# Aazmp/vp8oclenc

Measured on AMD Instinct MI355X. Metric: macroblocks/sec inter-frame (ME+DCT+loopfilter), 1080p, higher is better.
Workload: dtype u8/int32

## Files before the change

### vp8oclenc_amd/build.py

```python
from __future__ import annotations

import os
import shutil
import subprocess

PKG = os.path.dirname(os.path.abspath(__file__))
CSRC = os.path.join(PKG, "csrc")
LIB = os.path.join(PKG, "libvp8hip.so")
SOURCES = ["api_context.hip", "api_inter.hip", "api_entropy.hip", "api_batch.hip", "api_shard.hip", "api_profile.hip", "kernels_me.hip", "kernels_scale.hip", "kernels_denoise.hip", "api_denoise.hip", "kernels_s2.hip", "kernels_mb.hip", "kernels_lf3.hip", "kernels_lf4.hip", "kernels_lf_simple.hip", "kernels_quality.hip", "api_quality.hip", "kernels_entropy_stage.hip", "kernels_rc.hip", "kernels_intra.hip", "vp8_host.cpp", "vp8_driver.cpp", "vp8_bitstream.cpp"]
HEADERS = ["vp8hip_ctx.h", "vp8hip_dev.h", "kernels_rc_dev.h", "lf_shared.h", "lf_banded.h", "vp8_rfc6386_tables.inc", "vp8_mbhdr.h", "kernels_ent.hip", "kernels_hdr.hip"]
HEADERS = HEADERS + [os.path.join("..", "..", "include", h) for h in ("vp8hip.h", "vp8hip_multi.h", "vp8hip_taps.h", "vp8hip_host.h", "vp8hip_driver.h", "vp8hip_bitstream.h")]


def _hipcc() -> str:
    for cand in (shutil.which("hipcc"), "/opt/rocm/bin/hipcc"):
        if cand and os.path.exists(cand):
            return cand
    raise RuntimeError("hipcc not found: the MI355X path cannot be built (there is no CPU fallback)")


def stale() -> bool:
    if not os.path.exists(LIB):
        return True
    t = os.path.getmtime(LIB)
    deps = [os.path.join(CSRC, s) for s in SOURCES] + [os.path.normpath(os.path.join(CSRC, h)) for h in HEADERS]
    return any(os.path.exists(d) and os.path.getmtime(d) > t for d in deps)


def build(force: bool = False, verbose: bool = False) -> str:
    if not force and not stale():
        return LIB
    objs = []
    procs = []
    odir = os.path.join(PKG, "build")
    os.makedirs(odir, exist_ok=True)
    flags = ["--offload-arch=gfx950", "-O3", "-fPIC", "-std=c++17", "-ffp-contract=off", "-Wall", "-Wno-unused-function", "-Wno-bitwise-instead-of-logical", "-Wno-unused-value", "-Wno-missing-braces",
             "-I", os.path.join(PKG, "..", "include")] + os.environ.get("VP8HIP_EXTRA_FLAGS", "").split()
    for src in SOURCES:
        path = os.path.join(CSRC, src)
        if not os.path.exists(path):
            continue
        obj = os.path.join(odir, os.path.splitext(src)[0] + ".o")
        objs.append(obj)
        cmd = [_hipcc()] + flags + (["-x", "hip"] if src.endswith(".hip") else []) + ["-c", path, "-o", obj]
        if verbose:
            print(" ".join(cmd))
        procs.append((src, subprocess.Popen(cmd, stdout=subprocess.PIPE, stderr=subprocess.STDOUT, text=True)))
    for src, p in procs:
        out, _ = p.communicate()
        if p.returncode != 0:
            raise RuntimeError(f"hipcc failed on {src}:\n{out}")
        if verbose and out.strip():
            print(out)
    cmd = [_hipcc(), "--offload-arch=gfx950", "-shared", "-fPIC", "-o", LIB] + objs + ["-ldl", "-lpthread"]
    r = subprocess.run(cmd, stdout=subprocess.PIPE, stderr=subprocess.STDOUT, text=True)
    if r.returncode != 0:
        raise RuntimeError(f"link failed:\n{r.stdout}")
    return LIB


if __name__ == "__main__":
    print(build(force=True, verbose=True))
```

### vp8oclenc_amd/csrc/api_batch.hip

```cpp
#include "vp8hip_ctx.h"

using namespace vp8;

namespace vp8 {

bool batch_ent_stream(vp8hip_batch *b) {
    static const int mode = [] { const char *v = getenv("VP8HIP_BATCH_ENT_STREAM"); return v && v[0] ? atoi(v) : 0; }();
    if (!b->ev_ent && (hipEventCreateWithFlags(&b->ev_ent_fork, hipEventDisableTiming) != hipSuccess ||
                       hipEventCreateWithFlags(&b->ev_ent, FRAME_EVENT_FLAGS) != hipSuccess))
        return false;
    if (!mode) return false;
    if (b->ent) return true;
    int least = 0, greatest = 0;
    if (mode >= 2 && hipDeviceGetStreamPriorityRange(&least, &greatest) == hipSuccess) {
        if (hipStreamCreateWithPriority(&b->ent, hipStreamNonBlocking, mode == 3 ? greatest : least) != hipSuccess) b->ent = nullptr;
    } else if (hipStreamCreateWithFlags(&b->ent, hipStreamNonBlocking) != hipSuccess) {
        b->ent = nullptr;
    }
    return b->ent != nullptr;
}

}

extern "C" {


int vp8hip_batch_create(vp8hip_batch **out, vp8hip_ctx *const *ctxs, int n) {
    if (!out || !ctxs || n < 1 || n > MAX_BATCH) return VP8HIP_ERR_ARG;
    *out = nullptr;
    for (int i = 0; i < n; ++i) {
        if (!ctxs[i] || ctxs[i]->W != ctxs[0]->W || ctxs[i]->H != ctxs[0]->H || ctxs[i]->device != ctxs[0]->device ||
            ctxs[i]->ssim_target != ctxs[0]->ssim_target || ctxs[i]->lf_overlap || ctxs[i]->conformant != ctxs[0]->conformant ||
            !same_intake(ctxs[i], ctxs[0]))
            return VP8HIP_ERR_ARG;
        if (!ctxs[i]->own_stream) return VP8HIP_ERR_STATE;
        for (int j = 0; j < i; ++j)
            if (ctxs[j] == ctxs[i]) return VP8HIP_ERR_ARG;
    }
    vp8hip_batch *b = new (std::nothrow) vp8hip_batch();
    if (!b) return VP8HIP_ERR_ARG;
    USE_DEVICE(ctxs[0]);
    b->n = n;
    for (int i = 0; i < n; ++i) {
        hipStreamSynchronize(ctxs[i]->stream);
        if (ctxs[i]->own_stream) hipStreamDestroy(ctxs[i]->own_stream);
        ctxs[i]->own_stream = nullptr;
    }
    if (hipStreamCreateWithFlags(&b->stream, hipStreamNonBlocking) != hipSuccess) {
        for (int i = 0; i < n; ++i) {
            hipStreamCreateWithFlags(&ctxs[i]->own_stream, hipStreamNonBlocking);
            ctxs[i]->stream = ctxs[i]->own_stream;
        }
        delete b;
        return VP8HIP_ERR_HIP;
    }
    for (int i = 0; i < n; ++i) {
        ctxs[i]->stream = b->stream;
        ctxs[i]->batch = b;
        b->c[i] = ctxs[i];
        if (ctxs[i]->counted) --g_live_contexts;
        ctxs[i]->counted = false;
    }
    ++g_live_contexts;
    const int prep_mode = vp8hip_batch_prep_mode();
    bool ok = true;
    if (prep_mode) {
        ok = hipEventCreateWithFlags(&b->ev_gate, hipEventDisableTiming) == hipSuccess &&
             hipEventCreateWithFlags(&b->ev_gate2, hipEventDisableTiming) == hipSuccess &&
             hipEventCreateWithFlags(&b->ev_prep, hipEventDisableTiming) == hipSuccess;
        int least = 0, greatest = 0;
        ok = ok && hipDeviceGetStreamPriorityRange(&least, &greatest) == hipSuccess;
        static const bool normal_priority = getenv("VP8HIP_BATCH_PREP_PRIO") != nullptr;
        if (normal_priority) least = 0;
        if (ok && prep_mode == 2) {
            static hipStream_t shared[64] = {};
            hipStream_t &sh = shared[ctxs[0]->device & 63];
            if (!sh) ok = hipStreamCreateWithPriority(&sh, hipStreamNonBlocking, least) == hipSuccess;
            b->prep = sh;
            b->prep_shared = true;
        } else if (ok) {
            ok = hipStreamCreateWithPriority(&b->prep, hipStreamNonBlocking, least) == hipSuccess;
        }
    }
    if (!ok) {
        vp8hip_batch_destroy(b);
        return VP8HIP_ERR_HIP;
    }
    *out = b;
    return VP8HIP_OK;
}

void vp8hip_batch_destroy(vp8hip_batch *b) {
    if (!b) return;
    hipSetDevice(b->c[0]->device);
    if (b->prep) hipStreamSynchronize(b->prep);
    hipStreamSynchronize(b->stream);
    hipStreamDestroy(b->stream);
    if (b->prep && !b->prep_shared) hipStreamDestroy(b->prep);
    if (b->ev_gate) hipEventDestroy(b->ev_gate);
    if (b->ev_gate2) hipEventDestroy(b->ev_gate2);
    if (b->ev_prep) hipEventDestroy(b->ev_prep);
    if (b->ent) {
        hipStreamSynchronize(b->ent);
        hipStreamDestroy(b->ent);
    }
    if (b->copy) {
        hipStreamSynchronize(b->copy);
        hipStreamDestroy(b->copy);
        hipEventDestroy(b->ev_copied);
        hipEventDestroy(b->ev_packed[0]);
        hipEventDestroy(b->ev_packed[1]);
        for (int i = 0; i < b->n; ++i) { hipFree(b->stage[i][0]); hipFree(b->stage[i][1]); }
    }
    if (b->ev_ent_fork) hipEventDestroy(b->ev_ent_fork);
    if (b->ev_ent) hipEventDestroy(b->ev_ent);
    for (int i = 0; i < b->n; ++i) b->c[i]->frame_event = nullptr;
    --g_live_contexts;
    for (int i = 0; i < b->n; ++i) {
        b->c[i]->batch = nullptr;
        if (!b->c[i]->own_stream) hipStreamCreateWithFlags(&b->c[i]->own_stream, hipStreamNonBlocking);
        b->c[i]->stream = b->c[i]->own_stream;
        if (!b->c[i]->counted) ++g_live_contexts;
        b->c[i]->counted = true;
    }
    delete b;
}

static int stage_copy(vp8hip_batch *b, uint8_t *d, const void *y, const void *u, const void *v, size_t ny, size_t nc) {
    vp8hip_ctx *c0 = b->c[0];
    const uint8_t *py = static_cast<const uint8_t *>(y);
    if (u == py + ny && v == py + ny + nc) {
        HIPCHK(c0, hipMemcpyAsync(d, y, ny + 2 * nc, hipMemcpyHostToDevice, b->copy));
        return VP8HIP_OK;
    }
    HIPCHK(c0, hipMemcpyAsync(d, y, ny, hipMemcpyHostToDevice, b->copy));
    HIPCHK(c0, hipMemcpyAsync(d + ny, u, nc, hipMemcpyHostToDevice, b->copy));
    HIPCHK(c0, hipMemcpyAsync(d + ny + nc, v, nc, hipMemcpyHostToDevice, b->copy));
    return VP8HIP_OK;
}

static int batch_stage_ready(vp8hip_batch *b) {
    vp8hip_ctx *c0 = b->c[0];
    int sw, sh;
    incoming_size(c0, &sw, &sh);
    const size_t bytes = (size_t)sw * sh + 2 * (size_t)(sw / 2) * (sh / 2);
    if (!b->copy) {
        HIPCHK(c0, hipStreamCreateWithFlags(&b->copy, hipStreamNonBlocking));
        HIPCHK(c0, hipEventCreateWithFlags(&b->ev_copied, hipEventDisableTiming));
        HIPCHK(c0, hipEventCreateWithFlags(&b->ev_packed[0], hipEventDisableTiming));
        HIPCHK(c0, hipEventCreateWithFlags(&b->ev_packed[1], hipEventDisableTiming));
    }
    if (b->stage_bytes == bytes) return VP8HIP_OK;
    HIPCHK(c0, hipStreamSynchronize(b->copy));
    HIPCHK(c0, hipStreamSynchronize(b->stream));
    if (b->prep) HIPCHK(c0, hipStreamSynchronize(b->prep));
    for (int i = 0; i < b->n; ++i)
        for (int k = 0; k < 2; ++k) {
            (void)hipFree(b->stage[i][k]);
            b->stage[i][k] = nullptr;
            HIPCHK(c0, hipMalloc(&b->stage[i][k], bytes));
        }
    b->stage_bytes = bytes;
    b->packed_valid[0] = b->packed_valid[1] = false;
    b->pre_valid = false;
    return VP8HIP_OK;
}

static int batch_set_current(vp8hip_batch *b, const int *active, const void *const *y, const void *const *u, const void *const *v, bool host) {
    if (!b || !y || !u || !v) return VP8HIP_ERR_ARG;
    vp8hip_ctx *c0 = b->c[0];
    USE_DEVICE_ONLY(c0);
    const void *sy[MAX_BATCH], *su[MAX_BATCH], *sv[MAX_BATCH];
    int slot = -1;
    for (int i = 0; i < b->n; ++i) {
        if (active && !active[i]) continue;
        if (!y[i] || !u[i] || !v[i]) return VP8HIP_ERR_ARG;
        if (!same_intake(b->c[i], c0)) return VP8HIP_ERR_ARG;
    }
    if (host) {
        const int rc = batch_stage_ready(b);
        if (rc) return rc;
        int sw, sh;
        incoming_size(c0, &sw, &sh);
        const size_t ny = (size_t)sw * sh, nc = (size_t)(sw / 2) * (sh / 2);
        slot = b->stage_idx ^= 1;
        bool waited = false;
        for (int i = 0; i < b->n; ++i) {
            if (active && !active[i]) continue;
            uint8_t *d = b->stage[i][slot];
            if (!(b->pre_valid && b->pre[i][0] == y[i] && b->pre[i][1] == u[i] && b->pre[i][2] == v[i])) {
                if (!waited && b->packed_valid[slot]) HIPCHK(c0, hipStreamWaitEvent(b->copy, b->ev_packed[slot], 0));
                waited = true;
                {
                    const int cr = stage_copy(b, d, y[i], u[i], v[i], ny, nc);
                    if (cr) {
                        b->stage_idx ^= 1;
                        b->pre_valid = false;
                        return cr;
                    }
                }
            }
            sy[i] = d; su[i] = d + ny; sv[i] = d + ny + nc;
        }
        b->pre_valid = false;
        HIPCHK(c0, hipEventRecord(b->ev_copied, b->copy));
        y = sy; u = su; v = sv;
    }
    const Frame *f[MAX_BATCH];
    const void *py[MAX_BATCH], *pu[MAX_BATCH], *pv[MAX_BATCH];
    const ScalePlan *plans[MAX_BATCH];
    int n = 0;
    for (int i = 0; i < b->n; ++i) {
        if (active && !active[i]) continue;
        flush_scan(b->c[i]);
        next_current(b->c[i]);
        f[n] = &b->c[i]->cur;
        plans[n] = &b->c[i]->scale;
        py[n] = y[i]; pu[n] = u[i]; pv[n] = v[i];
        ++n;
    }
    if (!n) return VP8HIP_OK;
    hipStream_t ps = b->stream;
    if (b->prep) {
        HIPCHK(c0, hipStreamWaitEvent(b->prep, b->ev_gate, 0));
        HIPCHK(c0, hipEventRecord(b->ev_gate2, b->stream));
        hipEvent_t t_ = b->ev_gate;
        b->ev_gate = b->ev_gate2;
        b->ev_gate2 = t_;
        b->prep_pending = true;
        ps = b->prep;
    }
    if (host) HIPCHK(c0, hipStreamWaitEvent(ps, b->ev_copied, 0));
    {
        Timed t(c0, VP8HIP_K_PACK);
        if (c0->scale.in_w) launch_scale_batch(ps, f, py, pu, pv, plans, n);
        else launch_pack_batch(ps, f, py, pu, pv, n, c0->src_w, c0->src_h);
    }
    {
        DenoiseItem dn[MAX_BATCH];
        int nd = 0;
        for (int i = 0; i < b->n; ++i) {
            if (active && !active[i]) continue;
            if (denoise_item(b->c[i], ps, dn[nd])) ++nd;
        }
        launch_denoise_batch(ps, dn, nd, c0->dn_level);
    }
    HIPCHK(c0, hipGetLastError());
    if (host) {
        HIPCHK(c0, hipEventRecord(b->ev_packed[slot], ps));
        b->packed_valid[slot] = true;
    }
    return VP8HIP_OK;
}

int vp8hip_batch_set_current_device(vp8hip_batch *b, const int *active, const void *const *y, const void *const *u, const void *const *v) {
    return batch_set_current(b, active, y, u, v, false);
}

int vp8hip_batch_prefetch_current(vp8hip_batch *b, const uint8_t *const *y, const uint8_t *const *u, const uint8_t *const *v) {
    if (!b || !y || !u || !v) return VP8HIP_ERR_ARG;
    vp8hip_ctx *c0 = b->c[0];
    USE_DEVICE_ONLY(c0);
    const int rc = batch_stage_ready(b);
    if (rc) return rc;
    int sw, sh;
    incoming_size(c0, &sw, &sh);
    const size_t ny = (size_t)sw * sh, nc = (size_t)(sw / 2) * (sh / 2);
    const int slot = b->stage_idx ^ 1;
    if (b->packed_valid[slot]) HIPCHK(c0, hipStreamWaitEvent(b->copy, b->ev_packed[slot], 0));
    for (int i = 0; i < b->n; ++i) {
        b->pre[i][0] = b->pre[i][1] = b->pre[i][2] = nullptr;
        if (!y[i] || !u[i] || !v[i]) continue;
        uint8_t *d = b->stage[i][slot];
        { const int cr = stage_copy(b, d, y[i], u[i], v[i], ny, nc); if (cr) return cr; }
        b->pre[i][0] = y[i]; b->pre[i][1] = u[i]; b->pre[i][2] = v[i];
    }
    HIPCHK(c0, hipEventRecord(b->ev_copied, b->copy));
    b->pre_valid = true;
    return VP8HIP_OK;
}

int vp8hip_batch_upload_current(vp8hip_batch *b, const int *active, const uint8_t *const *y, const uint8_t *const *u, const uint8_t *const *v) {
    if (!b) return VP8HIP_ERR_ARG;
    if (b->copy) {
        (void)hipSetDevice(b->c[0]->device);
        HIPCHK(b->c[0], hipEventSynchronize(b->ev_copied));
    }
    return batch_set_current(b, active, reinterpret_cast<const void *const *>(y), reinterpret_cast<const void *const *>(u),
                             reinterpret_cast<const void *const *>(v), true);
}

int vp8hip_batch_auto_segments(vp8hip_batch *b, const int *active, const int *is_key_frame, const int32_t (*refqi)[4], int qi_min) {
    if (!b || !is_key_frame || !refqi) return VP8HIP_ERR_ARG;
    vp8hip_ctx *c0 = b->c[0];
    USE_DEVICE_ONLY(c0);
    const Frame *cur[MAX_BATCH];
    uint32_t *partial[MAX_BATCH], *stats[MAX_BATCH];
    SegData *sd[MAX_BATCH];
    int32_t *strength[MAX_BATCH];
    int key[MAX_BATCH];
    int32_t qi[MAX_BATCH][4];
    int n = 0;
    for (int i = 0; i < b->n; ++i) {
        if (active && !active[i]) continue;
        vp8hip_ctx *c = b->c[i];
        if (c->cur_count == 0) return VP8HIP_ERR_STATE;
        next_params(c);
        cur[n] = &c->cur;
        partial[n] = c->d_stats + 8;
        stats[n] = c->d_stats;
        sd[n] = c->d_sd;
        strength[n] = reinterpret_cast<int32_t *>(c->d_stats + 4);
        key[n] = is_key_frame[i] ? 1 : 0;
        for (int k = 0; k < 4; ++k) qi[n][k] = refqi[i][k];
        ++n;
    }
    static const bool own_launch = [] { const char *v = getenv("VP8HIP_BATCH_SCAN_LAUNCH"); return v && v[0] == '1'; }();
    if (n && !b->prep && !own_launch) {
        int k = 0;
        for (int i = 0; i < b->n; ++i) {
            if (active && !active[i]) continue;
            vp8hip_ctx *c = b->c[i];
            c->scan_req = ScanRequest{partial[k], stats[k], sd[k], strength[k], key[k], {qi[k][0], qi[k][1], qi[k][2], qi[k][3]}, qi_min};
            c->scan_deferred = true;
            ++k;
        }
        return VP8HIP_OK;
    }
    if (n && b->prep) b->prep_pending = true;
    if (n) launch_auto_segments_batch(b->prep ? b->prep : b->stream, cur, partial, stats, sd, strength, key, qi, qi_min, n);
    HIPCHK(c0, hipGetLastError());
    return VP8HIP_OK;
}

int vp8hip_batch_inter_transform(vp8hip_batch *b, const int *active, const int *prev_is_golden, const int *prev_is_altref,
                                 const int *use_golden, const int *use_altref) {
    if (!b || !prev_is_golden || !prev_is_altref || !use_golden || !use_altref) return VP8HIP_ERR_ARG;
    vp8hip_ctx *c0 = b->c[0];
    USE_DEVICE_ONLY(c0);
    vp8hip_ctx *m[MAX_BATCH];
    RefSet refs[MAX_BATCH];
    const Frame *cur[MAX_BATCH], *recon[MAX_BATCH], *pyr[2 * MAX_BATCH], *pyr_cur[MAX_BATCH];
    const ScanRequest *scans[MAX_BATCH] = {};
    int npyr_cur = 0;
    const NetSet *nets[MAX_BATCH];
    const MBOut *outs[MAX_BATCH];
    const SegData *sds[MAX_BATCH];
    int n = 0, npyr = 0;
    uint32_t pyr_border = 0;
    for (int i = 0; i < b->n; ++i) {
        if (active && !active[i]) continue;
        if (b->c[i]->conformant != c0->conformant) return VP8HIP_ERR_ARG;
        const int rc = inter_check(b->c[i], prev_is_golden[i], prev_is_altref[i], use_golden[i], use_altref[i]);
        if (rc) return rc;
    }
    for (int i = 0; i < b->n; ++i) {
        if (active && !active[i]) continue;
        vp8hip_ctx *c = b->c[i];
        const int rc = inter_begin(c, prev_is_golden[i], prev_is_altref[i], use_golden[i], use_altref[i]);
        if (rc) {
            for (int k = 0; k < n; ++k)
                if (scans[k]) m[k]->scan_deferred = true;
            return rc;
        }
        FrameSurf &last = c->frames[c->slot[0]];
        if (!c->cur_pyramid_valid) {
            if (b->prep) pyr_cur[npyr_cur++] = &c->cur;
            else pyr[npyr++] = &c->cur;
        }
        bool border_alone = false;
        if (!last.pyramid_valid) {
            if (!last.border_valid) pyr_border |= 1u << npyr;
            pyr[npyr++] = &last.f;
        } else if (!last.border_valid) {
            border_alone = true;
        }
        if (border_alone) {
            batch_join_prep(b);
            launch_border(b->stream, last.f);
        }
        last.pyramid_valid = true;
        last.border_valid = true;
        c->cur_pyramid_valid = true;
        refs[n] = ref_set(c, 1, use_golden[i], use_altref[i]);
        cur[n] = &c->cur;
        recon[n] = &c->frames[c->recon].f;
        nets[n] = &c->nets;
        outs[n] = &c->out;
        sds[n] = c->d_sd;
        if (c->scan_deferred) {
            scans[n] = &c->scan_req;
            c->scan_deferred = false;
        }
        m[n++] = c;
    }
    if (!n) return VP8HIP_OK;
    hipStream_t s = b->stream;
    if (npyr_cur) {
        b->prep_pending = true;
        launch_pyramid_batch(b->prep, pyr_cur, npyr_cur, 0);
    }
    batch_join_prep(b);
    if (npyr) {
        Timed t(c0, VP8HIP_K_DOWNSAMPLE);
        launch_pyramid_batch(s, pyr, npyr, pyr_border);
    }
    const int net_width = c0->mbw * 2;
    static const int coarse_mode = [] { const char *v = getenv("VP8HIP_BATCH_S1_COARSE"); return v && v[0] ? atoi(v) : 0; }();
    int first_level = 4, src = 0;
    if (coarse_mode > 0 && c0->mbw >= 2 && c0->mbh >= 2) {
        Timed t(c0, VP8HIP_K_SEARCH1_L2);
        if (launch_search1_coarse_batch(s, cur, refs, nets, net_width, n, coarse_mode == 2, coarse_mode == 3)) {
            first_level = coarse_mode == 2 ? -1 : (coarse_mode == 3 ? 1 : 0);
            src = first_level == 1 ? 1 : 0;
        }
    }
    for (int l = first_level; l >= 0; --l) {
        Timed t(c0, VP8HIP_K_SEARCH1_L4 + (4 - l));
        launch_search1_batch(s, cur, refs, nets, l, src, net_width, n);
        src ^= 1;
    }
    bool carried;
    {
        Timed t(c0, VP8HIP_K_SEARCH2);
        carried = launch_search2_batch(s, cur, refs, nets, n, s2_clock(c0), scans);
    }
    for (int i = 0; i < n && !carried; ++i)
        if (scans[i]) launch_auto_segments(s, m[i]->cur, scans[i]->partial, scans[i]->stats, scans[i]->sd, scans[i]->strength_out, scans[i]->is_key,
                                           scans[i]->refqi, scans[i]->qi_min);
    {
        Timed t(c0, VP8HIP_K_MB);
        launch_mb_batch(s, cur, refs, nets, recon, outs, sds, c0->ssim_target, c0->mbw, c0->mbh, n, c0->conformant != 0);
    }
    for (int i = 0; i < n; ++i) m[i]->recon_ready = true, m[i]->recon_key = false;
    HIPCHK(c0, hipGetLastError());
    return VP8HIP_OK;
}

int vp8hip_batch_loop_filter(vp8hip_batch *b, const int *active) {
    if (!b) return VP8HIP_ERR_ARG;
    vp8hip_ctx *c0 = b->c[0];
    USE_DEVICE(c0);
    vp8hip_ctx *m[MAX_BATCH];
    const Frame *recon[MAX_BATCH];
    const MBOut *outs[MAX_BATCH];
    SegData *sds[MAX_BATCH];
    int32_t *prog[MAX_BATCH];
    void *hand[MAX_BATCH];
    unsigned launch_no[MAX_BATCH];
    LfCheck chk[MAX_BATCH];
    int n = 0, type = -1;
    for (int i = 0; i < b->n; ++i) {
        if (active && !active[i]) continue;
        if (!b->c[i]->recon_ready || b->c[i]->recon < 0) return VP8HIP_ERR_STATE;
        if (type >= 0 && b->c[i]->lf_type != type) return VP8HIP_ERR_STATE;
        type = b->c[i]->lf_type;
    }
    for (int i = 0; i < b->n; ++i) {
        if (active && !active[i]) continue;
        vp8hip_ctx *c = b->c[i];
        recon[n] = &c->frames[c->recon].f;
        outs[n] = &c->out;
        sds[n] = c->d_sd;
        prog[n] = c->d_progress;
        hand[n] = c->d_lf_handoff;
        launch_no[n] = type == 1 ? c->lf_simple_launches++ : c->lf_launches++;
        lf_check(c, chk[n]);
        c->verdict_stream = b->stream;
        m[n++] = c;
    }
    if (!n) return VP8HIP_OK;
    if (b->ent) HIPCHK(c0, hipEventRecord(b->ev_ent_fork, b->stream));
    {
        Timed t(c0, VP8HIP_K_LOOP_FILTER);
        static const bool form4 = [] { const char *v = getenv("VP8HIP_LF_BATCH_FORM"); return v && atoi(v) == 4; }();
        if (type == 1) launch_loop_filter_simple_batch(b->stream, recon, outs, sds, prog, c0->mbw, c0->mbh, launch_no, n, chk);
        else if (form4) launch_loop_filter4_batch(b->stream, recon, outs, sds, prog, hand, c0->mbw, c0->mbh, launch_no, n, chk);
        else launch_loop_filter3_batch(b->stream, recon, outs, sds, prog, c0->mbw, c0->mbh, launch_no, n, chk);
    }
    b->ent_fork_fresh = b->ent != nullptr;
    for (int i = 0; i < n; ++i) {
        vp8hip_ctx *c = m[i];
        c->frames[c->recon].pyramid_valid = false;
        c->frames[c->recon].border_valid = false;
        c->slot[0] = c->recon;
        c->lf_key = c->recon_key;
        c->recon = -1;
        c->recon_ready = false;
    }
    HIPCHK(c0, hipGetLastError());
    return batch_quality(b, active);
}

int vp8hip_batch_intra_transform(vp8hip_batch *b, const int *active) {
    if (!b) return VP8HIP_ERR_ARG;
    vp8hip_ctx *c0 = b->c[0];
    USE_DEVICE(c0);
    for (int i = 0; i < b->n; ++i) {
        if (active && !active[i]) continue;
        if (b->c[i]->cur_count == 0) return VP8HIP_ERR_STATE;
    }
    CheckItem it[MAX_BATCH];
    vp8hip_ctx *m[MAX_BATCH];
    int n = 0;
    for (int i = 0; i < b->n; ++i) {
        if (active && !active[i]) continue;
        vp8hip_ctx *c = b->c[i];
        const int rc = claim_recon(c);
        if (rc) return rc;
        c->ent_counted_partitions = 0;
        drop_overflowed_frame(c);
        ++c->out_gen;
        CheckItem &k = it[n];
        k.cur = &c->cur;
        k.recon = &c->frames[c->recon].f;
        k.o = &c->out;
        k.sd = c->d_sd;
        k.modes = c->intra_modes;
        k.is_inter = c->intra_is_inter;
        k.prog = c->intra_prog;
        k.err = c->d_progress + LF_ERR_WORD;
        k.gen = ++c->intra_gen;
        m[n++] = c;
    }
    if (!n) return VP8HIP_OK;
    {
        Timed t(c0, VP8HIP_K_INTRA);
        launch_intra_key_batch(b->stream, it, n, c0->mbw, c0->mbh);
    }
    {
        Timed t(c0, VP8HIP_K_FILTER_MASK);
        for (int i = 0; i < n; ++i) launch_filter_mask(b->stream, m[i]->out, m[i]->d_sd, m[i]->mbs);
    }
    for (int i = 0; i < n; ++i) m[i]->recon_ready = true, m[i]->recon_key = true;
    HIPCHK(c0, hipGetLastError());
    return VP8HIP_OK;
}

int vp8hip_batch_check_ssim_async(vp8hip_batch *b, const int *active, const int32_t (*refqi)[4], int qi_min) {
    if (!b || !refqi) return VP8HIP_ERR_ARG;
    vp8hip_ctx *c0 = b->c[0];
    USE_DEVICE(c0);
    for (int i = 0; i < b->n; ++i) {
        if (active && !active[i]) continue;
        const vp8hip_ctx *c = b->c[i];
        if (!c->recon_ready || c->recon < 0 || c->cur_count == 0 || c->verdict_pending || c->chk_armed) return VP8HIP_ERR_STATE;
    }
    CheckItem it[MAX_BATCH];
    int n = 0;
    for (int i = 0; i < b->n; ++i) {
        if (active && !active[i]) continue;
        check_item(b->c[i], it[n++], refqi[i], qi_min);
    }
    if (!n) return VP8HIP_OK;
    if (fallback_possible(c0->ssim_target)) {
        Timed t(c0, VP8HIP_K_INTRA);
        launch_check_fallback(b->stream, it, n, c0->ssim_target, c0->mbw, c0->mbh, c0->conformant);
    }
    HIPCHK(c0, hipGetLastError());
    return VP8HIP_OK;
}

int vp8hip_batch_encode_frame_begin(vp8hip_batch *b, const int *active, int num_partitions, const vp8hip_header_params *params) {
    if (!b || !params) return VP8HIP_ERR_ARG;
    const int P = num_partitions;
    if (P != 1 && P != 2 && P != 4 && P != 8) return VP8HIP_ERR_ARG;
    vp8hip_ctx *c0 = b->c[0];
    bool early = b->ent_fork_fresh;
    USE_DEVICE(c0);
    FrameEntropy e[MAX_BATCH];
    FrameOut fo[MAX_BATCH];
    vp8hip_ctx *m[MAX_BATCH];
    int n = 0;
    for (int i = 0; i < b->n; ++i) {
        if (active && !active[i]) continue;
        if (b->c[i]->frame_pending) return VP8HIP_ERR_STATE;
    }
    for (int i = 0; i < b->n; ++i) {
        if (active && !active[i]) continue;
        vp8hip_ctx *c = b->c[i];
        const int rc = frame_prepare(c, P, &params[i], e[n], fo[n]);
        if (rc) return rc;
        c->frame_params = params[i];
        c->frame_partitions = P;
        m[n++] = c;
    }
    if (!n) return VP8HIP_OK;
    const bool side = !c0->prof_mask && batch_ent_stream(b);
    hipStream_t s = side ? b->ent : b->stream;
    if (side) {
        for (int i = 0; i < n; ++i) early = early && !m[i]->verdict_pending;
        if (!early) HIPCHK(c0, hipEventRecord(b->ev_ent_fork, b->stream));
        HIPCHK(c0, hipStreamWaitEvent(b->ent, b->ev_ent_fork, 0));
    }
    {
        Timed t(c0, VP8HIP_K_ENT_COUNT);
        launch_fe_count_batch(s, e, n);
    }
    {
        Timed t(c0, VP8HIP_K_HDR_ENCODE);
        launch_fe_emit_batch(s, e, n);
    }
    {
        Timed t(c0, VP8HIP_K_ENT_ENCODE);
        launch_frame_code_batch(s, e, fo, n);
    }
    HIPCHK(c0, hipGetLastError());
    for (int i = 0; i < n; ++i) {
        vp8hip_ctx *c = m[i];
        c->ent_counted_partitions = P;
        if (!frame_zero_copy()) {
            const size_t first = c->h_frame_cap < FRAME_FIRST_COPY ? c->h_frame_cap : FRAME_FIRST_COPY;
            HIPCHK(c0, hipMemcpyAsync(c->h_frame, c->d_frame, first, hipMemcpyDeviceToHost, s));
        }
        c->frame_pending = true;
        c->frame_gen = c->out_gen;
        c->frame_event = b->ev_ent;
    }
    if (b->ev_ent) HIPCHK(c0, hipEventRecord(b->ev_ent, s));
    if (side) HIPCHK(c0, hipStreamWaitEvent(b->stream, b->ev_ent, 0));
    return VP8HIP_OK;
}

}
```

### vp8oclenc_amd/csrc/api_profile.hip

```cpp
#include "vp8hip_ctx.h"

using namespace vp8;

namespace vp8 {

int prof_collect(vp8hip_ctx *c) {
    if (c->ev_used == 0) return VP8HIP_OK;
    HIPCHK(c, hipStreamSynchronize(c->stream));
    for (int i = 0; i < c->ev_used; i += 2) {
        float ms = 0;
        HIPCHK(c, hipEventElapsedTime(&ms, c->ev[i], c->ev[i + 1]));
        c->prof_ms[c->ev_kernel[i / 2]] += ms;
        c->prof_n[c->ev_kernel[i / 2]] += 1;
    }
    c->ev_used = 0;
    return VP8HIP_OK;
}

}

extern "C" {

int vp8hip_profile_enable(vp8hip_ctx *c, uint32_t mask) {
    USE_DEVICE(c);
    JOIN_LF(c);
    if (!c) return VP8HIP_ERR_ARG;
    int rc = prof_collect(c);
    c->prof_mask = mask;
    return rc;
}

int vp8hip_profile_read(vp8hip_ctx *c, double *total_ms, int64_t *launches) {
    USE_DEVICE(c);
    if (!c) return VP8HIP_ERR_ARG;
    int rc = prof_collect(c);
    if (rc) return rc;
    for (int k = 0; k < VP8HIP_K_COUNT; ++k) {
        if (total_ms) total_ms[k] = c->prof_ms[k];
        if (launches) launches[k] = c->prof_n[k];
        c->prof_ms[k] = 0;
        c->prof_n[k] = 0;
    }
    return VP8HIP_OK;
}

int vp8hip_profile_read_clock(vp8hip_ctx *c, double *loop_filter_ms, int64_t *loop_filter_launches, double *shader_clock_ghz) {
    USE_DEVICE(c);
    if (!c || !loop_filter_ms || !loop_filter_launches) return VP8HIP_ERR_ARG;
    JOIN_LF(c);
    unsigned long long clk[6] = {0, 0, 0, 0, 0, 0};
    int32_t *base = c->d_progress + LF_ERR_WORD + 4;
    HIPCHK(c, hipMemcpyAsync(clk, base, sizeof(clk), hipMemcpyDeviceToHost, c->stream));
    HIPCHK(c, hipMemsetAsync(base + 2, 0, 40, c->stream));
    HIPCHK(c, hipStreamSynchronize(c->stream));
    c->lf_context_switches = (int64_t)clk[5];
    if (getenv("VP8HIP_DEBUG_CLOCK")) fprintf(stderr, "lf clock: launches %llu anomalies %llu hw_id changed %llu\n", clk[2], clk[4], clk[5]);
    *loop_filter_ms = (double)clk[1] * 1e-5;
    *loop_filter_launches = (int64_t)clk[2];
    if (shader_clock_ghz) *shader_clock_ghz = clk[2] > clk[4] ? (double)clk[3] / (double)(clk[2] - clk[4]) * 1e-4 : 0.0;
    return VP8HIP_OK;
}

int vp8hip_profile_search2_clock(vp8hip_ctx *c, int on) {
    if (!c) return VP8HIP_ERR_ARG;
    c->s2_clock_on = on != 0;
    return VP8HIP_OK;
}

int vp8hip_profile_read_search2_clock(vp8hip_ctx *c, double *ms, int64_t *launches) {
    USE_DEVICE(c);
    if (!c || !ms || !launches) return VP8HIP_ERR_ARG;
    JOIN_LF(c);
    unsigned long long w[5] = {0, 0, 0, 0, 0};
    HIPCHK(c, hipMemcpyAsync(w, s2_clock_words(c), sizeof(w), hipMemcpyDeviceToHost, c->stream));
    HIPCHK(c, hipMemsetAsync(s2_clock_words(c) + 3, 0, 16, c->stream));
    HIPCHK(c, hipStreamSynchronize(c->stream));
    *ms = (double)w[3] * 1e-5;
    *launches = (int64_t)w[4];
    return VP8HIP_OK;
}

int64_t vp8hip_profile_context_switches(const vp8hip_ctx *c) { return c ? c->lf_context_switches : 0; }

int vp8hip_debug_download(vp8hip_ctx *c, int what, int ref, int level, void *dst, size_t bytes) {
    USE_DEVICE(c);
    JOIN_LF(c);
    if (!c || !dst) return VP8HIP_ERR_ARG;
    hipStream_t s = c->stream;
    switch (what) {
        case VP8HIP_DBG_NET1:
        case VP8HIP_DBG_NET2: {
            if (ref < 0 || ref > 2 || bytes != (size_t)c->b8 * 4) return VP8HIP_ERR_ARG;
            HIPCHK(c, hipMemcpyAsync(dst, c->nets.net[ref][what == VP8HIP_DBG_NET1 ? 0 : 1], bytes, hipMemcpyDeviceToHost, s));
            break;
        }
        case VP8HIP_DBG_BDIFF:
            if (ref < 0 || ref > 2 || bytes != (size_t)c->b8 * 4) return VP8HIP_ERR_ARG;
            HIPCHK(c, hipMemcpyAsync(dst, c->nets.bdiff[ref], bytes, hipMemcpyDeviceToHost, s));
            break;
        case VP8HIP_DBG_PYRAMID: {
            if (ref < 0 || ref > 3 || level < 0 || level > 4) return VP8HIP_ERR_ARG;
            if (ref < 3 && c->slot[ref] < 0) return VP8HIP_ERR_STATE;
            const Frame &f = ref == 3 ? c->cur : c->frames[c->slot[ref]].f;
            const Plane &p = f.Y[level];
            if (bytes != (size_t)p.w * p.h) return VP8HIP_ERR_ARG;
            int rc = copy_out(c, dst, p);
            if (rc) return rc;
            break;
        }
        case VP8HIP_DBG_MB_MASK:
        case VP8HIP_DBG_MB_NZ:
            if (bytes != (size_t)c->mbs * 4) return VP8HIP_ERR_ARG;
            HIPCHK(c, hipMemcpyAsync(dst, what == VP8HIP_DBG_MB_MASK ? c->out.mask : c->out.nz, bytes, hipMemcpyDeviceToHost, s));
            break;
        case VP8HIP_DBG_THIRD_CONTEXT:
            if (bytes != (size_t)c->mbs * 25) return VP8HIP_ERR_ARG;
            HIPCHK(c, hipMemcpyAsync(dst, c->ent_third, bytes, hipMemcpyDeviceToHost, s));
            break;
        case VP8HIP_DBG_CURRENT_CHROMA: {
            if (ref < 0 || ref > 1 || c->cur_count == 0) return VP8HIP_ERR_ARG;
            const Plane &p = ref ? c->cur.V : c->cur.U;
            if (bytes != (size_t)p.w * p.h) return VP8HIP_ERR_ARG;
            int rc = copy_out(c, dst, p);
            if (rc) return rc;
            break;
        }
        case 100:
            if (bytes != 512) return VP8HIP_ERR_ARG;
            HIPCHK(c, hipMemcpyAsync(dst, (const char *)c->d_progress + 4096, 512, hipMemcpyDeviceToHost, s));
            break;
        default:
            return VP8HIP_ERR_ARG;
    }
    HIPCHK(c, hipStreamSynchronize(s));
    return VP8HIP_OK;
}

int vp8hip_debug_weight(vp8hip_ctx *c, const int32_t *d, int n, int32_t *out) {
    USE_DEVICE(c);
    JOIN_LF(c);
    if (!c || !d || !out || n <= 0) return VP8HIP_ERR_ARG;
    int32_t *dd = nullptr, *dout = nullptr;
    HIPCHK(c, hipMalloc(&dd, (size_t)n * 64));
    HIPCHK(c, hipMalloc(&dout, (size_t)n * 4));
    HIPCHK(c, hipMemcpyAsync(dd, d, (size_t)n * 64, hipMemcpyHostToDevice, c->stream));
    launch_weight_tap(c->stream, dd, n, dout);
    HIPCHK(c, hipMemcpyAsync(out, dout, (size_t)n * 4, hipMemcpyDeviceToHost, c->stream));
    HIPCHK(c, hipStreamSynchronize(c->stream));
    hipFree(dd);
    hipFree(dout);
    return VP8HIP_OK;
}

int vp8hip_debug_weight_mfma(vp8hip_ctx *c, const int32_t *d, int n, int32_t *out) {
    USE_DEVICE(c);
    JOIN_LF(c);
    if (!c || !d || !out || n <= 0) return VP8HIP_ERR_ARG;
    int32_t *dd = nullptr, *dout = nullptr;
    HIPCHK(c, hipMalloc(&dd, (size_t)n * 64));
    HIPCHK(c, hipMalloc(&dout, (size_t)n * 4));
    HIPCHK(c, hipMemcpyAsync(dd, d, (size_t)n * 64, hipMemcpyHostToDevice, c->stream));
    launch_weight_tap_mfma(c->stream, dd, n, dout);
    HIPCHK(c, hipMemcpyAsync(out, dout, (size_t)n * 4, hipMemcpyDeviceToHost, c->stream));
    HIPCHK(c, hipStreamSynchronize(c->stream));
    hipFree(dd);
    hipFree(dout);
    return VP8HIP_OK;
}

int vp8hip_debug_lf_stall(vp8hip_ctx *c, int on) {
    USE_DEVICE(c);
    JOIN_LF(c);
    if (!c) return VP8HIP_ERR_ARG;
    c->lf_stall_test = on ? 1 : 0;
    return VP8HIP_OK;
}

int vp8hip_debug_upload_ssim(vp8hip_ctx *c, const float *ssim) {
    USE_DEVICE(c);
    JOIN_LF(c);
    if (!c || !ssim) return VP8HIP_ERR_ARG;
    HIPCHK(c, hipMemcpyAsync(c->out.ssim, ssim, (size_t)c->mbs * 4, hipMemcpyHostToDevice, c->stream));
    HIPCHK(c, hipStreamSynchronize(c->stream));
    return VP8HIP_OK;
}

int vp8hip_debug_upload_header_inputs(vp8hip_ctx *c, const int32_t *seg, const int32_t *nz, const int32_t *ref, const int32_t *parts,
                                      const int16_t *vectors, const int32_t *is_inter, const int32_t *modes, const uint32_t *probs,
                                      const uint32_t *denom, const int32_t *sd) {
    USE_DEVICE(c);
    JOIN_LF(c);
    if (!c) return VP8HIP_ERR_ARG;
    hipStream_t s = c->stream;
    const size_t n = c->mbs;
    if (seg) HIPCHK(c, hipMemcpyAsync(c->out.seg, seg, n * 4, hipMemcpyHostToDevice, s));
    if (nz) HIPCHK(c, hipMemcpyAsync(c->out.nz, nz, n * 4, hipMemcpyHostToDevice, s));
    if (ref) HIPCHK(c, hipMemcpyAsync(c->out.ref, ref, n * 4, hipMemcpyHostToDevice, s));
    if (parts) HIPCHK(c, hipMemcpyAsync(c->out.parts, parts, n * 4, hipMemcpyHostToDevice, s));
    if (vectors) HIPCHK(c, hipMemcpyAsync(c->out.vec, vectors, n * 16, hipMemcpyHostToDevice, s));
    if (is_inter) HIPCHK(c, hipMemcpyAsync(c->intra_is_inter, is_inter, n * 4, hipMemcpyHostToDevice, s));
    if (modes) HIPCHK(c, hipMemcpyAsync(c->intra_modes, modes, n * 64, hipMemcpyHostToDevice, s));
    if (probs) HIPCHK(c, hipMemcpyAsync(c->ent_probs, probs, sizeof(uint32_t) * ENT_NCTX, hipMemcpyHostToDevice, s));
    if (denom) HIPCHK(c, hipMemcpyAsync(c->ent_denom0, denom, sizeof(uint32_t) * ENT_NCTX, hipMemcpyHostToDevice, s));
    if (sd) HIPCHK(c, hipMemcpyAsync(c->d_sd, sd, sizeof(SegData), hipMemcpyHostToDevice, s));
    HIPCHK(c, hipStreamSynchronize(s));
    if (probs || denom) c->ent_counted_partitions = 1;
    return VP8HIP_OK;
}

}
```

### vp8oclenc_amd/csrc/kernels_lf3.hip

```cpp
#include "lf_banded.h"

namespace vp8 {

namespace lf3 {

using namespace lfb;

struct NormalFilter {
    static constexpr bool CHROMA = true;
    static constexpr bool LEVEL0_ENDS_PLANE = true;
    typedef int4 Lim;
    static __device__ __forceinline__ Lim limits(const int32_t *sd) {
        const int il = sd[SD_INTERIOR_LIMIT] & 0xff;
        return make_int4(il, il - (sd[SD_MBEDGE_LIMIT] & 0xff) * 2 - 1, il - (sd[SD_SUB_BEDGE_LIMIT] & 0xff) * 2 - 1, sd[SD_HEV_THRESHOLD] & 0xff);
    }
    struct Step { Limits L; int int_lim, il4, il8; };
    static __device__ __forceinline__ Step step(const Lim &lim, bool inner, bool luma) {
        Step s;
        s.int_lim = lim.x;
        s.L.mb_delta = lim.y;
        s.L.b_delta = lim.z;
        s.L.hev_thr = lim.w;
        s.il4 = inner ? s.int_lim : -1;
        s.il8 = inner && luma ? s.int_lim : -1;
        return s;
    }
    static __device__ __forceinline__ void line(int (&t)[20], const Step &s, bool mb_edge) { filter_line(t, s.L, mb_edge ? s.int_lim : -1, s.il4, s.il8); }
};

__global__ __launch_bounds__(NWAVES * 64) void k_loop_filter3_b(BatchOf<Args> b) { loop_filter_body<NormalFilter>(b.item[blockIdx.z]); }

}

static bool lf_skip() {
    static const bool skip = experiment_skip("lf");
    return skip;
}

void launch_loop_filter3_batch(hipStream_t s, const Frame *const *recon, const MBOut *const *o, SegData *const *d_sd,
                               int32_t *const *progress, int mbw, int mbh, const unsigned *launch_no, int n, const LfCheck *chk) {
    lfb::launch_batch(lf3::k_loop_filter3_b, s, recon, o, d_sd, progress, 0, mbw, mbh, launch_no, n, chk, lf_skip());
}

}
```

### vp8oclenc_amd/csrc/kernels_lf_simple.hip

```cpp
#include "lf_banded.h"

namespace vp8 {

namespace lfs {

using namespace lfb;

__device__ __forceinline__ void simple_edge(int &p0, int &q0, int p1, int q1, int lim2) {
    const int sum = (int)__builtin_amdgcn_sad_u16((uint32_t)p1, (uint32_t)q1, (uint32_t)(ad(p0, q0) << 2));
    int w = c128(c128(p1 - q1) + __mul24(q0 - p0, 3));
    w = sum <= lim2 ? w : 0;
    w = imin(w, 123);
    q0 = satb(q0 - ((w + 4) >> 3));
    p0 = satb(p0 + ((w + 3) >> 3));
}

__device__ __forceinline__ void simple_line(int (&t)[20], int lim2_mb, int lim2_in) {
#pragma unroll
    for (int k = 4; k < 20; k += 4) simple_edge(t[k - 1], t[k], t[k - 2], t[k + 1], k == 4 ? lim2_mb : lim2_in);
}

struct SimpleFilter {
    static constexpr bool CHROMA = false;
    static constexpr bool LEVEL0_ENDS_PLANE = false;
    typedef int2 Lim;
    static __device__ __forceinline__ Lim limits(const int32_t *sd) {
        const bool on = sd[SD_LOOP_FILTER_LEVEL] != 0;
        return make_int2(on ? (sd[SD_MBEDGE_LIMIT] & 0xff) * 2 + 1 : -1, on ? (sd[SD_SUB_BEDGE_LIMIT] & 0xff) * 2 + 1 : -1);
    }
    struct Step { int lim_mb, lim_in; };
    static __device__ __forceinline__ Step step(const Lim &lim, bool inner, bool) { return Step{lim.x, inner ? lim.y : -1}; }
    static __device__ __forceinline__ void line(int (&t)[20], const Step &s, bool mb_edge) { simple_line(t, mb_edge ? s.lim_mb : -1, s.lim_in); }
};

__global__ __launch_bounds__(NWAVES * 64) void k_loop_filter_simple(Args a) { loop_filter_body<SimpleFilter>(a); }
__global__ __launch_bounds__(NWAVES * 64) void k_loop_filter_simple_b(BatchOf<Args> b) { loop_filter_body<SimpleFilter>(b.item[blockIdx.z]); }

}

bool loop_filter_simple_fits(int mbh) { return (mbh + 1 + lfb::ROWS - 1) / lfb::ROWS + 1 <= LF_SIMPLE_WORDS; }

void launch_loop_filter_simple(hipStream_t s, const Frame &recon, const MBOut &o, SegData *d_sd, int32_t *progress, int mbw, int mbh,
                               unsigned launch_no, const LfCheck *chk) {
    const lfb::Args a = lfb::make_args(s, recon, o, d_sd, progress, LF_SIMPLE_WORD, mbw, mbh, launch_no, chk);
    VP8_LAUNCH(lfs::k_loop_filter_simple, dim3(a.nbands + (a.chk.on ? 1 : 0)), dim3(lfb::NWAVES * 64), 0, s, a);
}

void launch_loop_filter_simple_batch(hipStream_t s, const Frame *const *recon, const MBOut *const *o, SegData *const *d_sd,
                                     int32_t *const *progress, int mbw, int mbh, const unsigned *launch_no, int n, const LfCheck *chk) {
    lfb::launch_batch(lfs::k_loop_filter_simple_b, s, recon, o, d_sd, progress, LF_SIMPLE_WORD, mbw, mbh, launch_no, n, chk);
}

}
```

### vp8oclenc_amd/csrc/kernels_me.hip

```cpp
#include <stdlib.h>
#include <string.h>

#include "vp8hip_dev.h"

namespace vp8 {

struct BorderItem { Plane y, u, v; };
static_assert(EXT == 8, "border_row stores a margin as one eight-byte word");
__device__ __forceinline__ void border_row(const Plane &pl, int row, int lane) {
    if (row >= pl.h + EXT) return;
    uint8_t *dst = pl.p + (ptrdiff_t)row * pl.stride;
    const uint8_t *src = pl.p + (ptrdiff_t)iclamp(row, 0, pl.h - 1) * pl.stride;
    if (row < 0 || row >= pl.h)
        for (int x = lane * 8; x < pl.w; x += 512) *reinterpret_cast<uint2 *>(dst + x) = *reinterpret_cast<const uint2 *>(src + x);
    if (lane < 2) {
        const uint32_t s4 = (uint32_t)src[lane ? pl.w - 1 : 0] * 0x01010101u;
        *reinterpret_cast<uint2 *>(dst + (lane ? pl.w : -EXT)) = make_uint2(s4, s4);
    }
}
__device__ __forceinline__ void border_body(const BorderItem &a) {
    border_row(blockIdx.y == 0 ? a.y : (blockIdx.y == 1 ? a.u : a.v), (int)blockIdx.x - EXT, threadIdx.x);
}

__global__ __launch_bounds__(64) void k_border(BorderItem a) { border_body(a); }

void launch_border(hipStream_t s, const Frame &f) {
    dim3 grid(f.Y[0].h + 2 * EXT, 3);
    VP8_LAUNCH(k_border, grid, dim3(64), 0, s, BorderItem{f.Y[0], f.U, f.V});
}

struct PyrArgs { Frame f[2 * MAX_BATCH]; uint32_t border_mask; };
static int border_jobs(const Frame &f) { return (f.Y[0].h + 2 * EXT) + 2 * (f.U.h + 2 * EXT); }

__global__ __launch_bounds__(256) void k_pyramid(PyrArgs a) {
    __shared__ uint8_t s2[16][16];
    __shared__ uint8_t s3[8][8];
    const Frame &f = a.f[blockIdx.z];
    const int t = threadIdx.x, tx = t & 15, ty = t >> 4;
    const Plane &P0 = f.Y[0];
    const int tiles_y = (P0.h + 63) / 64;
    const int tile = xcd_band((int)blockIdx.y * (int)gridDim.x + (int)blockIdx.x, tiles_y * (int)gridDim.x);
    const int bx = tile % (int)gridDim.x, by = tile / (int)gridDim.x;
    if ((int)blockIdx.y >= tiles_y) {
        if (!((a.border_mask >> blockIdx.z) & 1)) return;
        int job = (((int)blockIdx.y - tiles_y) * (int)gridDim.x + (int)blockIdx.x) * 4 + (t >> 6);
        const int ny = P0.h + 2 * EXT, nc = f.U.h + 2 * EXT;
        if (job < ny) border_row(P0, job - EXT, t & 63);
        else if (job < ny + nc) border_row(f.U, job - ny - EXT, t & 63);
        else if (job < ny + 2 * nc) border_row(f.V, job - ny - nc - EXT, t & 63);
        return;
    }
    const int sx = imin(bx * 64 + 4 * tx, P0.w - 4), sy0 = by * 64 + 4 * ty;
    uint32_t r[4];
#pragma unroll
    for (int k = 0; k < 4; ++k)
        r[k] = *reinterpret_cast<const uint32_t *>(P0.p + (ptrdiff_t)imin(sy0 + k, P0.h - 1) * P0.stride + sx);
    int l1[2][2];
#pragma unroll
    for (int j = 0; j < 2; ++j)
#pragma unroll
        for (int i = 0; i < 2; ++i)
            l1[j][i] = (byte_of(r[2 * j], 2 * i) + byte_of(r[2 * j], 2 * i + 1) + byte_of(r[2 * j + 1], 2 * i) +
                        byte_of(r[2 * j + 1], 2 * i + 1) + 2) >> 2;
    const Plane &P1 = f.Y[1];
    const int x1 = bx * 32 + 2 * tx, y1 = by * 32 + 2 * ty;
    if (x1 < P1.w) {
#pragma unroll
        for (int j = 0; j < 2; ++j)
            if (y1 + j < P1.h)
                *reinterpret_cast<uint16_t *>(P1.p + (ptrdiff_t)(y1 + j) * P1.stride + x1) = (uint16_t)(l1[j][0] | (l1[j][1] << 8));
    }
    const int l2 = (l1[0][0] + l1[0][1] + l1[1][0] + l1[1][1] + 2) >> 2;
    const Plane &P2 = f.Y[2];
    const int x2 = bx * 16 + tx, y2 = by * 16 + ty;
    if (x2 < P2.w && y2 < P2.h) P2.p[(ptrdiff_t)y2 * P2.stride + x2] = (uint8_t)l2;
    s2[ty][tx] = (uint8_t)l2;
    __syncthreads();
    if (t < 64) {
        const int ux = t & 7, uy = t >> 3;
        const int l3 = (s2[2 * uy][2 * ux] + s2[2 * uy][2 * ux + 1] + s2[2 * uy + 1][2 * ux] + s2[2 * uy + 1][2 * ux + 1] + 2) >> 2;
        const Plane &P3 = f.Y[3];
        const int x3 = bx * 8 + ux, y3 = by * 8 + uy;
        if (x3 < P3.w && y3 < P3.h) P3.p[(ptrdiff_t)y3 * P3.stride + x3] = (uint8_t)l3;
        s3[uy][ux] = (uint8_t)l3;
    }
    __syncthreads();
    if (t < 16) {
        const int ux = t & 3, uy = t >> 2;
        const int l4 = (s3[2 * uy][2 * ux] + s3[2 * uy][2 * ux + 1] + s3[2 * uy + 1][2 * ux] + s3[2 * uy + 1][2 * ux + 1] + 2) >> 2;
        const Plane &P4 = f.Y[4];
        const int x4 = bx * 4 + ux, y4 = by * 4 + uy;
        if (x4 < P4.w && y4 < P4.h) P4.p[(ptrdiff_t)y4 * P4.stride + x4] = (uint8_t)l4;
    }
}

static dim3 pyramid_grid(const Frame &f, int nframes, uint32_t border_mask) {
    const int gx = (f.Y[0].w + 63) / 64, gy = (f.Y[0].h + 63) / 64;
    const int extra = border_mask ? ((border_jobs(f) + 3) / 4 + gx - 1) / gx : 0;
    return dim3(gx, gy + extra, nframes);
}
void launch_pyramid(hipStream_t s, const Frame *a, const Frame *b, uint32_t border_mask) {
    PyrArgs p;
    p.f[0] = *a;
    p.f[1] = b ? *b : *a;
    p.border_mask = border_mask;
    VP8_LAUNCH(k_pyramid, pyramid_grid(*a, b ? 2 : 1, border_mask), dim3(256), 0, s, p);
}
void launch_pyramid_batch(hipStream_t s, const Frame *const *f, int nframes, uint32_t border_mask) {
    if (nframes <= 0) return;
    PyrArgs p;
    for (int i = 0; i < nframes; ++i) p.f[i] = *f[i];
    p.border_mask = border_mask;
    VP8_LAUNCH(k_pyramid, pyramid_grid(*f[0], nframes, border_mask), dim3(256), 0, s, p);
}

struct PackItem { Plane py, pu, pv; const uint8_t *sy, *su, *sv; int sw, sh, ssy, ssc; };
__device__ __forceinline__ void pack_body(const PackItem &a, int per) {
    const Plane &py = a.py, &pu = a.pu, &pv = a.pv;
    const uint8_t *sy = a.sy, *su = a.su, *sv = a.sv;
    const int ny = (py.w >> 3) * py.h, nc = (pu.w >> 3) * pu.h;
    for (int k = 0; k < per; ++k) {
        int i = ((int)blockIdx.x * per + k) * 256 + (int)threadIdx.x;
        const Plane *pl = &py;
        const uint8_t *src = sy;
        int sw = a.sw, sh = a.sh, ss = a.ssy;
        if (i >= ny) {
            i -= ny;
            pl = &pu;
            src = su;
            sw >>= 1; sh >>= 1; ss = a.ssc;
            if (i >= nc) { i -= nc; pl = &pv; src = sv; }
            if (i >= nc) return;
        }
        const int upr = pl->w >> 3;
        const int y = i / upr, x = (i % upr) * 8;
        const uint8_t *row = src + (size_t)(y < sh ? y : sh - 1) * ss;
        uint2 v;
        if (x + 8 <= sw && ((ss | (int)(reinterpret_cast<uintptr_t>(src) & 7)) & 7) == 0) {
            v = *reinterpret_cast<const uint2 *>(row + x);
        } else {
            uint32_t w[2] = {0, 0};
#pragma unroll
            for (int j = 0; j < 8; ++j) w[j >> 2] |= (uint32_t)row[x + j < sw ? x + j : sw - 1] << (8 * (j & 3));
            v = make_uint2(w[0], w[1]);
        }
        *reinterpret_cast<uint2 *>(pl->p + (ptrdiff_t)y * pl->stride + x) = v;
    }
}

__global__ __launch_bounds__(256) void k_pack_b(BatchOf<PackItem> b, int per) { pack_body(b.item[blockIdx.z], per); }
static int pack_units_per_thread() {
    static const int per = [] { const char *e = getenv("VP8HIP_PACK_UNITS"); const int v = e ? atoi(e) : 16; return v < 1 ? 1 : (v > 64 ? 64 : v); }();
    return per;
}

static PackItem pack_item(const Frame &f, const void *y, const void *u, const void *v, int sw, int sh, int ssy, int ssc) {
    if (sw <= 0) { sw = f.Y[0].w; sh = f.Y[0].h; }
    if (ssy <= 0) { ssy = sw; ssc = sw >> 1; }
    return PackItem{f.Y[0], f.U, f.V, (const uint8_t *)y, (const uint8_t *)u, (const uint8_t *)v, sw, sh, ssy, ssc};
}
void launch_pack(hipStream_t s, const Frame &f, const void *y, const void *u, const void *v, int sw, int sh, int ssy, int ssc) {
    const int n = (f.Y[0].w >> 3) * f.Y[0].h + 2 * ((f.U.w >> 3) * f.U.h);
    BatchOf<PackItem> b;
    b.n = 1;
    b.item[0] = pack_item(f, y, u, v, sw, sh, ssy, ssc);
    const int per = pack_units_per_thread();
    VP8_LAUNCH(k_pack_b, dim3((n + 256 * per - 1) / (256 * per), 1, 1), dim3(256), 0, s, b, per);
}
void launch_pack_batch(hipStream_t s, const Frame *const *f, const void *const *y, const void *const *u, const void *const *v, int n,
                       int sw, int sh) {
    BatchOf<PackItem> b;
    b.n = n;
    for (int i = 0; i < n; ++i) b.item[i] = pack_item(*f[i], y[i], u[i], v[i], sw, sh, 0, 0);
    const int units = (f[0]->Y[0].w >> 3) * f[0]->Y[0].h + 2 * ((f[0]->U.w >> 3) * f[0]->U.h);
    static const bool skip = experiment_skip("pack");
    if (skip) return;
    const int per = pack_units_per_thread();
    VP8_LAUNCH(k_pack_b, dim3((units + 256 * per - 1) / (256 * per), 1, n), dim3(256), 0, s, b, per);
}

struct Search1Args {
    Plane cur;
    Plane ref[3];
    const int16_t *src[3];
    int16_t *dst[3];
    int refmap[3];
    int nrefs;
    int net_width, w, h, pixel_rate, rate_shift, nblk, bw;
    int pbw, pbh;
    uint32_t bw_inv;
};

template <bool SPLIT>
struct S1Map {
    static constexpr int LANES_PER_BLOCK = SPLIT ? 20 : 5;
    static constexpr int BLOCKS_PER_WAVE = SPLIT ? 3 : 12;
    static constexpr int BLOCKS_PER_WG = 4 * BLOCKS_PER_WAVE;
};

__device__ __forceinline__ void s1_subblock(const uint8_t *cp, int cstride, const uint8_t *rp, int rstride, int acc[5]) {
    uint32_t c[4], q0[4], q1[4];
#pragma unroll
    for (int y = 0; y < 4; ++y) {
        c[y] = *reinterpret_cast<const uint32_t *>(cp + (ptrdiff_t)y * cstride) ^ 0x80808080u;
        const uint2 q = ld_u64(rp + (ptrdiff_t)y * rstride);
        q0[y] = q.x ^ 0x80808080u; q1[y] = q.y ^ 0x80808080u;
    }
    uint32_t cc[4], col[8];
    transpose4x4(c, cc);
    transpose4x4(q0, col);
    transpose4x4(q1, col + 4);
    int pre[16];
#pragma unroll
    for (int k = 0; k < 4; ++k) weight_pre_column(cc[k], pre + 4 * k);
#pragma unroll
    for (int i = 0; i < 5; ++i) acc[i] += weight_cols_pre(pre, col + i);
}

__device__ __forceinline__ int vcopy(uint32_t x) {
    int y;
    asm volatile("v_mov_b32 %0, %1" : "=v"(y) : "v"(x));
    return y;
}
__device__ __forceinline__ void s1_subblock_pre(v4i wa, const int *pre_lds, int pre_off, const uint8_t *rp, int rstride, int acc[5]) {
    uint32_t q0[4], q1[4];
#pragma unroll
    for (int y = 0; y < 4; ++y) {
        const uint2 q = ld_u64(rp + (ptrdiff_t)y * rstride);
        q0[y] = q.x ^ 0x80808080u; q1[y] = q.y ^ 0x80808080u;
    }
    uint32_t col[8];
    transpose4x4(q0, col);
    transpose4x4(q1, col + 4);
#pragma unroll
    for (int i = 0; i < 5; ++i) {
        int off = pre_off;
        asm volatile("" : "+v"(off));
        __builtin_amdgcn_sched_barrier(0);
        const v4i b = (i & 1) ? v4i{vcopy(col[i]), vcopy(col[i + 1]), vcopy(col[i + 2]), vcopy(col[i + 3])}
                              : v4i{(int)col[i], (int)col[i + 1], (int)col[i + 2], (int)col[i + 3]};
        acc[i] += weight_mfma(wa, load_pre16(pre_lds + off), b);
    }
}
constexpr int S1_PRE_INTS = 12 * 4 * 16;
__device__ __forceinline__ void s1_make_pre(const Plane &cur, int cx, int cy, int sb, bool on, int *dst16) {
    const int sx = (sb >> 1) * 4, sy = (sb & 1) * 4;
    const uint8_t *cp = cur.p + (ptrdiff_t)(cy + sy) * cur.stride + cx + sx;
    uint32_t c[4], cc[4];
#pragma unroll
    for (int y = 0; y < 4; ++y) c[y] = *reinterpret_cast<const uint32_t *>(cp + (ptrdiff_t)y * cur.stride) ^ 0x80808080u;
    transpose4x4(c, cc);
    int pre[16];
    weight_pre_block(cc, pre);
    if (on) {
#pragma unroll
        for (int k = 0; k < 4; ++k) *reinterpret_cast<int4 *>(dst16 + 4 * k) = make_int4(pre[4 * k], pre[4 * k + 1], pre[4 * k + 2], pre[4 * k + 3]);
    }
}

template <bool SPLIT, bool PRE_LDS = false>
__device__ __forceinline__ uint32_t search1_block(const Search1Args &a, int r, int cx, int cy, uint32_t pv, bool live, int sub, int lane,
                                                  const int *pre_lds = nullptr ,
                                                  int pre_off = 0 ) {
    const int sb0 = sub / 5, j = sub - 5 * sb0;
    int v0x = (int16_t)(pv & 0xffffu), v0y = (int16_t)(pv >> 16);
    const int rmask = a.pixel_rate - 1;
    v0x = (v0x + ((v0x >> 31) & rmask)) >> a.rate_shift;
    v0y = (v0y + ((v0y >> 31) & rmask)) >> a.rate_shift;
    if (a.pixel_rate > 8) v0x = v0y = 0;

    const int py = (int16_t)(cy + v0y + (j - 2));
    const bool row_valid = live && py >= 0 && py <= a.h - 8;
    const int xb = cx + v0x - 2;
    const bool loadable = row_valid && xb >= -8 && xb <= a.w - 4;
    const int lx = loadable ? xb : cx, ly = loadable ? py : cy;

    const uint8_t *cp = a.cur.p + (ptrdiff_t)cy * a.cur.stride + cx;
    const uint8_t *rp = a.ref[r].p + (ptrdiff_t)ly * a.ref[r].stride + lx;
    int acc[5] = {0, 0, 0, 0, 0};
    if (SPLIT) {
        const int sx = (sb0 >> 1) * 4, sy = (sb0 & 1) * 4;
        s1_subblock(cp + (ptrdiff_t)sy * a.cur.stride + sx, a.cur.stride, rp + (ptrdiff_t)sy * a.ref[r].stride + sx, a.ref[r].stride, acc);
#pragma unroll
        for (int i = 0; i < 5; ++i) {
            acc[i] += __shfl(acc[i], lane + 10, 64);
            acc[i] += __shfl(acc[i], lane + 5, 64);
        }
    } else {
        if (PRE_LDS) {
            const v4i wa = metric_a(lane);
#pragma unroll 1
            for (int sb = 0; sb < 4; ++sb) {
                const int sx = (sb >> 1) * 4, sy = (sb & 1) * 4;
                s1_subblock_pre(wa, pre_lds, pre_off + 16 * sb, rp + (ptrdiff_t)sy * a.ref[r].stride + sx, a.ref[r].stride, acc);
            }
        } else {
#pragma unroll 1
            for (int sb = 0; sb < 4; ++sb) {
                const int sx = (sb >> 1) * 4, sy = (sb & 1) * 4;
                s1_subblock(cp + (ptrdiff_t)sy * a.cur.stride + sx, a.cur.stride, rp + (ptrdiff_t)sy * a.ref[r].stride + sx, a.ref[r].stride, acc);
            }
        }
    }
    const int pen_mask = a.pixel_rate < 4 ? -1 : 0;
    const int pen_y = iabs(iabs(py - cy) - v0y);
    uint32_t best = 0xffffffffu;
#pragma unroll
    for (int i = 0; i < 5; ++i) {
        const int px = (int16_t)(xb + i);
        const bool valid = loadable && px >= 0 && px <= a.w - 8;
        const int diff = (acc[i] + (((iabs(iabs(px - cx) - v0x) + pen_y) << 5) & pen_mask)) & 0xffff;
        const uint32_t key = (valid && diff < 0x7fff) ? ((uint32_t)diff << 8) | (uint32_t)(j * 5 + i) : 0xffffffffu;
        best = key < best ? key : best;
    }
#pragma unroll
    for (int off = 1; off <= 4; off <<= 1) {
        const uint32_t o = (uint32_t)__shfl((int)best, lane + off, 64);
        if (j + off < 5 && o < best) best = o;
    }
    int bx, by;
    if (best != 0xffffffffu) {
        const int k = best & 0xff;
        bx = v0x + (k % 5 - 2);
        by = v0y + (k / 5 - 2);
    } else {
        bx = (int16_t)(v0x - cx);
        by = (int16_t)(v0y - cy);
    }
    const uint32_t ox16 = (uint16_t)(int16_t)((int16_t)bx * (int16_t)a.pixel_rate);
    const uint32_t oy16 = (uint16_t)(int16_t)((int16_t)by * (int16_t)a.pixel_rate);
    return ox16 | (oy16 << 16);
}

template <bool SPLIT, bool PRE_LDS = false, bool REF_LOOP = false>
__device__ __forceinline__ void search1_body(const Search1Args &a) {
    using M = S1Map<SPLIT>;
    if (!REF_LOOP && (int)blockIdx.y >= a.nrefs) return;
    const int lane = threadIdx.x & 63, wave = threadIdx.x >> 6;
    const int grp = lane / M::LANES_PER_BLOCK, sub = lane - M::LANES_PER_BLOCK * grp;
    const int b_raw = (xcd_band(blockIdx.x, gridDim.x) * 4 + wave) * M::BLOCKS_PER_WAVE + grp;
    const bool live = grp < M::BLOCKS_PER_WAVE && b_raw < a.nblk;
    const int b = live ? b_raw : a.nblk - 1;
    const int by = a.bw == 1 ? b : (int)__umulhi((uint32_t)b, a.bw_inv), bx = b - by * a.bw;
    const int cx = bx * 8, cy = by * 8;
    const int parent = (cy >> 4) * a.net_width + (cx >> 4);
    const bool parent_written = (cx >> 4) < a.pbw && (cy >> 4) < a.pbh;
    const int *pre_lds = nullptr;
    int pre_off = 0;
    if (!SPLIT && PRE_LDS) {
        __shared__ __attribute__((aligned(16))) int s_pre[4][S1_PRE_INTS];
        const int slot = lane >> 2, sb = lane & 3;
        const int tb_raw = (xcd_band(blockIdx.x, gridDim.x) * 4 + wave) * M::BLOCKS_PER_WAVE + slot;
        const int tb = tb_raw < a.nblk ? tb_raw : a.nblk - 1;
        const int tby = a.bw == 1 ? tb : (int)__umulhi((uint32_t)tb, a.bw_inv), tbx = tb - tby * a.bw;
        s1_make_pre(a.cur, tbx * 8, tby * 8, sb, slot < M::BLOCKS_PER_WAVE, &s_pre[wave][(slot < M::BLOCKS_PER_WAVE ? slot : 0) * 64 + sb * 16]);
        asm volatile("s_waitcnt lgkmcnt(0)" ::: "memory");
        pre_lds = &s_pre[0][0];
        pre_off = wave * S1_PRE_INTS + (grp < M::BLOCKS_PER_WAVE ? grp : 0) * 64;
    }
    const int nr = REF_LOOP ? a.nrefs : 1;
#pragma unroll 1
    for (int ri = 0; ri < nr; ++ri) {
        const int r = a.refmap[REF_LOOP ? ri : (int)blockIdx.y];
        const uint32_t pv = parent_written ? reinterpret_cast<const uint32_t *>(a.src[r])[parent] : 0u;
        const uint32_t out = search1_block<SPLIT, !SPLIT && PRE_LDS>(a, r, cx, cy, pv, live, sub, lane, pre_lds, pre_off);
        if (sub == 0 && live) {
            const int cell = (cy >> 3) * a.net_width + (cx >> 3);
            reinterpret_cast<uint32_t *>(a.dst[r])[cell] = out;
        }
    }
}

struct CoarseArgs { Search1Args lv[5]; };
constexpr int COARSE_WAVES = 6;
template <bool FINEST, bool TOP_ONLY = false>
__device__ __forceinline__ void coarse_tile(const Search1Args &L0, const Search1Args &L1, const Search1Args &L2, const Search1Args &L3, const Search1Args &L4, int r) {
    using M = S1Map<true>;
    __shared__ uint32_t mv4, mv3, mv2[4], mv1[16];
    const int lane = threadIdx.x & 63, wave = threadIdx.x >> 6;
    const int grp = lane / M::LANES_PER_BLOCK, sub = lane - M::LANES_PER_BLOCK * grp;
    const int slot = grp < M::BLOCKS_PER_WAVE ? wave * M::BLOCKS_PER_WAVE + grp : 99;
    const int tiles_x = (L1.bw + 3) / 4;
    const int tile = xcd_band(blockIdx.x, gridDim.x);
    const int ty = tile / tiles_x, tx = tile - ty * tiles_x;
    {
        const int bx = tx >> 1, by = ty >> 1;
        const bool exists = bx < L4.bw && by * L4.bw + bx < L4.nblk;
        if (wave == 0) {
            const bool live = slot == 0 && exists;
            const uint32_t out = search1_block<true>(L4, r, (live ? bx : 0) * 8, (live ? by : 0) * 8, 0u, live, sub, lane);
            if (slot == 0 && sub == 0) mv4 = exists ? out : 0u;
        }
    }
    __syncthreads();
    {
        const bool exists = tx < L3.bw && ty * L3.bw + tx < L3.nblk;
        if (wave == 0) {
            const bool live = slot == 0 && exists;
            const uint32_t out = search1_block<true>(L3, r, (live ? tx : 0) * 8, (live ? ty : 0) * 8, mv4, live, sub, lane);
            if (slot == 0 && sub == 0) mv3 = exists ? out : 0u;
        }
    }
    __syncthreads();
    if (wave < 2) {
        const int i = slot & 1, j = (slot >> 1) & 1;
        const int bx = 2 * tx + i, by = 2 * ty + j;
        const bool exists = slot < 4 && bx < L2.bw && by * L2.bw + bx < L2.nblk;
        const uint32_t out = search1_block<true>(L2, r, (exists ? bx : 0) * 8, (exists ? by : 0) * 8, mv3, exists, sub, lane);
        if (slot < 4 && sub == 0) mv2[slot] = exists ? out : 0u;
        if (TOP_ONLY && slot < 4 && sub == 0 && exists) reinterpret_cast<uint32_t *>(L2.dst[r])[by * L2.net_width + bx] = out;
    }
    if (TOP_ONLY) return;
    __syncthreads();
    {
        const int i = slot & 3, j = (slot >> 2) & 3;
        const int bx = 4 * tx + i, by = 4 * ty + j;
        const bool live = slot < 16 && bx < L1.bw && by * L1.bw + bx < L1.nblk;
        const uint32_t pv = mv2[(((j >> 1) & 1) << 1) | ((i >> 1) & 1)];
        const uint32_t out = search1_block<true>(L1, r, (live ? bx : 0) * 8, (live ? by : 0) * 8, pv, live, sub, lane);
        if (sub == 0 && live) reinterpret_cast<uint32_t *>(L1.dst[r])[by * L1.net_width + bx] = out;
        if (FINEST && sub == 0 && slot < 16) mv1[slot] = live ? out : 0u;
    }
    if (!FINEST) return;
    __syncthreads();
    {
        using M0 = S1Map<false>;
        const int grp0 = lane / M0::LANES_PER_BLOCK, sub0 = lane - M0::LANES_PER_BLOCK * grp0;
        const int slot0 = grp0 < M0::BLOCKS_PER_WAVE ? wave * M0::BLOCKS_PER_WAVE + grp0 : 99;
        const int i = slot0 & 7, j = (slot0 >> 3) & 7;
        const int bx = 8 * tx + i, by = 8 * ty + j;
        const bool live = slot0 < 64 && bx < L0.bw && by * L0.bw + bx < L0.nblk;
        const uint32_t pv = mv1[((j >> 1) << 2) | (i >> 1)];
        const uint32_t out = search1_block<false>(L0, r, (live ? bx : 0) * 8, (live ? by : 0) * 8, pv, live, sub0, lane);
        if (sub0 == 0 && live) reinterpret_cast<uint32_t *>(L0.dst[r])[by * L0.net_width + bx] = out;
    }
}

template <bool FINEST>
__global__ __launch_bounds__(64 * COARSE_WAVES) void k_search1_coarse(CoarseArgs a) {
    if ((int)blockIdx.y >= a.lv[1].nrefs) return;
    coarse_tile<FINEST>(a.lv[0], a.lv[1], a.lv[2], a.lv[3], a.lv[4], a.lv[1].refmap[blockIdx.y]);
}

struct CoarseGeom { int w, h, cur_stride, ref_stride; };
struct CoarseMember {
    const uint8_t *cur[5];
    const uint8_t *ref[3][5];
    int16_t *dst1[3], *dst0[3];
    int refmap[3], nrefs;
};
struct CoarseBatchArgs { CoarseGeom g[5]; int net_width, n; CoarseMember m[MAX_BATCH]; };
static_assert(sizeof(CoarseBatchArgs) <= 4096, "a batch's argument block travels in the 4 KiB kernel-argument segment");
__device__ __forceinline__ Search1Args coarse_level(const CoarseBatchArgs &a, const CoarseMember &m, int l, int r) {
    Search1Args s;
    const CoarseGeom &g = a.g[l];
    s.cur = Plane{const_cast<uint8_t *>(m.cur[l]), g.cur_stride, g.w, g.h};
    s.ref[0] = Plane{const_cast<uint8_t *>(m.ref[r][l]), g.ref_stride, g.w, g.h};
    s.dst[0] = l == 1 ? m.dst1[r] : m.dst0[r];
    s.net_width = a.net_width;
    s.w = g.w;
    s.h = g.h;
    s.pixel_rate = 1 << l;
    s.rate_shift = l;
    s.bw = g.w / 8;
    s.nblk = (g.w / 8) * (g.h / 8);
    return s;
}
__global__ __launch_bounds__(128) void k_search1_top_b(CoarseBatchArgs a) {
    const CoarseMember &m = a.m[blockIdx.z];
    if ((int)blockIdx.y >= m.nrefs) return;
    const int r = m.refmap[blockIdx.y];
    const Search1Args L1 = coarse_level(a, m, 1, r), L2 = coarse_level(a, m, 2, r), L3 = coarse_level(a, m, 3, r), L4 = coarse_level(a, m, 4, r);
    coarse_tile<false, true>(L1, L1, L2, L3, L4, 0);
}
template <bool FINEST>
__global__ __launch_bounds__(64 * COARSE_WAVES) void k_search1_coarse_b(CoarseBatchArgs a) {
    const CoarseMember &m = a.m[blockIdx.z];
    if ((int)blockIdx.y >= m.nrefs) return;
    const int r = m.refmap[blockIdx.y];
    const Search1Args L0 = coarse_level(a, m, 0, r), L1 = coarse_level(a, m, 1, r), L2 = coarse_level(a, m, 2, r), L3 = coarse_level(a, m, 3, r),
                      L4 = coarse_level(a, m, 4, r);
    coarse_tile<FINEST>(L0, L1, L2, L3, L4, 0);
}

template <bool SPLIT>
__global__ __launch_bounds__(256) void k_search1(Search1Args a) { search1_body<SPLIT>(a); }
static_assert(sizeof(BatchOf<Search1Args>) <= 4096 && sizeof(PyrArgs) <= 4096 && sizeof(BatchOf<PackItem>) <= 4096, "a batch's argument blocks travel in the 4 KiB kernel-argument segment");
template <bool SPLIT>
__global__ __launch_bounds__(256) void k_search1_b(BatchOf<Search1Args> b) { search1_body<SPLIT>(b.item[blockIdx.z]); }
__global__ __attribute__((amdgpu_waves_per_eu(8, 8))) __launch_bounds__(256) void k_search1_pl(Search1Args a) { search1_body<false, true>(a); }
__global__ __attribute__((amdgpu_waves_per_eu(8, 8))) __launch_bounds__(256) void k_search1_pl_b(BatchOf<Search1Args> b) { search1_body<false, true>(b.item[blockIdx.z]); }
__global__ __attribute__((amdgpu_waves_per_eu(7, 8))) __launch_bounds__(256) void k_search1_plr_b(BatchOf<Search1Args> b) { search1_body<false, true, true>(b.item[blockIdx.z]); }
static bool search1_ref_loop() {
    static const bool on = [] { const char *v = getenv("VP8HIP_S1_REF_LOOP"); return !(v && v[0] == '0'); }();
    return on;
}
static bool search1_pre_lds() {
    static const bool on = [] { const char *v = getenv("VP8HIP_S1_PRE_LDS"); return !(v && v[0] == '0'); }();
    return on;
}

static Search1Args search1_args(const Frame &cur, const RefSet &refs, const NetSet &nets, int level, int src_idx, int net_width) {
    Search1Args a;
    a.cur = cur.Y[level];
    int n = 0;
    for (int r = 0; r < 3; ++r) {
        a.ref[r] = refs.ref[r].Y[level];
        a.src[r] = nets.net[r][src_idx];
        a.dst[r] = nets.net[r][src_idx ^ 1];
        if (refs.use[r]) a.refmap[n++] = r;
    }
    a.nrefs = n;
    for (int i = n; i < 3; ++i) a.refmap[i] = 0;
    a.net_width = net_width;
    a.w = a.cur.w;
    a.h = a.cur.h;
    a.pixel_rate = 1 << level;
    a.rate_shift = level;
    a.bw = a.w / 8;
    a.nblk = (a.w / 8) * (a.h / 8);
    a.bw_inv = a.bw > 0 ? (uint32_t)(((1ull << 32) + a.bw - 1) / a.bw) : 0;
    a.pbw = level < 4 ? cur.Y[level + 1].w / 8 : 0;
    a.pbh = level < 4 ? cur.Y[level + 1].h / 8 : 0;
    return a;
}

int persistent_workgroups() {
    static const int n = [] { const char *v = getenv("VP8HIP_PERSIST"); return v && v[0] ? atoi(v) : 0; }();
    return n;
}

static bool search1_skip() {
    static const bool skip = experiment_skip("s1");
    return skip;
}
static bool search1_split(size_t blocks_times_refs, bool latency) {
    static const int forced = [] { const char *v = getenv("VP8HIP_S1_SPLIT"); return v && v[0] ? (v[0] == '1' ? 1 : 0) : -1; }();
    return forced >= 0 ? forced == 1 : (latency || blocks_times_refs < (size_t)12 * 1024);
}

void launch_search1(hipStream_t s, const Frame &cur, const RefSet &refs, const NetSet &nets, int level, int src_idx,
                    int net_width, bool latency) {
    const Search1Args a = search1_args(cur, refs, nets, level, src_idx, net_width);
    const int n = a.nrefs;
    if (a.nblk <= 0 || n == 0 || search1_skip()) return;
    if (search1_split((size_t)a.nblk * n, latency))
        VP8_LAUNCH(k_search1<true>, dim3((a.nblk + S1Map<true>::BLOCKS_PER_WG - 1) / S1Map<true>::BLOCKS_PER_WG, n), dim3(256), 0, s, a);
    else if (search1_pre_lds())
        VP8_LAUNCH(k_search1_pl, dim3((a.nblk + S1Map<false>::BLOCKS_PER_WG - 1) / S1Map<false>::BLOCKS_PER_WG, n), dim3(256), 0, s, a);
    else
        VP8_LAUNCH(k_search1<false>, dim3((a.nblk + S1Map<false>::BLOCKS_PER_WG - 1) / S1Map<false>::BLOCKS_PER_WG, n), dim3(256), 0, s, a);
}

void launch_search1_coarse(hipStream_t s, const Frame &cur, const RefSet &refs, const NetSet &nets, int net_width, bool finest) {
    CoarseArgs a;
    for (int l = 0; l <= 4; ++l) a.lv[l] = search1_args(cur, refs, nets, l, l & 1, net_width);
    const Search1Args &L0 = a.lv[0], &L1 = a.lv[1];
    if (L0.nblk <= 0 || L0.nrefs == 0 || search1_skip()) return;
    const int tiles_x = finest ? (L0.bw + 7) / 8 : (L1.bw + 3) / 4, tiles_y = finest ? (L0.h / 8 + 7) / 8 : (L1.h / 8 + 3) / 4;
    if (tiles_x * tiles_y <= 0) return;
    if (finest) VP8_LAUNCH(k_search1_coarse<true>, dim3(tiles_x * tiles_y, L0.nrefs), dim3(64 * COARSE_WAVES), 0, s, a);
    else VP8_LAUNCH(k_search1_coarse<false>, dim3(tiles_x * tiles_y, L0.nrefs), dim3(64 * COARSE_WAVES), 0, s, a);
}

bool launch_search1_coarse_batch(hipStream_t s, const Frame *const *cur, const RefSet *refs, const NetSet *const *nets, int net_width, int n, bool finest, bool top_only) {
    CoarseBatchArgs a;
    a.net_width = net_width;
    a.n = n;
    int maxrefs = 0;
    for (int l = 0; l <= 4; ++l) {
        const Plane &c = cur[0]->Y[l];
        a.g[l] = CoarseGeom{c.w, c.h, c.stride, refs[0].ref[0].Y[l].stride};
    }
    for (int i = 0; i < n; ++i) {
        CoarseMember &m = a.m[i];
        int k = 0;
        for (int r = 0; r < 3; ++r) {
            for (int l = 0; l <= 4; ++l) {
                const Plane &rp = refs[i].ref[r].Y[l], &cp = cur[i]->Y[l];
                if (rp.stride != a.g[l].ref_stride || cp.stride != a.g[l].cur_stride || cp.w != a.g[l].w || cp.h != a.g[l].h || rp.w != cp.w || rp.h != cp.h) return false;
                m.ref[r][l] = rp.p;
                if (r == 0) m.cur[l] = cp.p;
            }
            m.dst1[r] = nets[i]->net[r][0];
            m.dst0[r] = nets[i]->net[r][1];
            if (refs[i].use[r]) m.refmap[k++] = r;
        }
        m.nrefs = k;
        for (int j = k; j < 3; ++j) m.refmap[j] = 0;
        maxrefs = k > maxrefs ? k : maxrefs;
    }
    const int bw0 = a.g[0].w / 8, bh0 = a.g[0].h / 8, bw1 = a.g[1].w / 8, bh1 = a.g[1].h / 8;
    if (bw0 * bh0 <= 0 || maxrefs == 0 || search1_skip()) return true;
    const int tiles_x = finest ? (bw0 + 7) / 8 : (bw1 + 3) / 4, tiles_y = finest ? (bh0 + 7) / 8 : (bh1 + 3) / 4;
    if (tiles_x * tiles_y <= 0) return !finest ? true : false;
    if (top_only) {
        VP8_LAUNCH(k_search1_top_b, dim3(tiles_x * tiles_y, maxrefs, n), dim3(128), 0, s, a);
        return true;
    }
    if (finest) VP8_LAUNCH(k_search1_coarse_b<true>, dim3(tiles_x * tiles_y, maxrefs, n), dim3(64 * COARSE_WAVES), 0, s, a);
    else VP8_LAUNCH(k_search1_coarse_b<false>, dim3(tiles_x * tiles_y, maxrefs, n), dim3(64 * COARSE_WAVES), 0, s, a);
    return true;
}

void launch_search1_batch(hipStream_t s, const Frame *const *cur, const RefSet *refs, const NetSet *const *nets, int level, int src_idx,
                          int net_width, int n) {
    BatchOf<Search1Args> b;
    b.n = n;
    int maxrefs = 0, totrefs = 0;
    for (int i = 0; i < n; ++i) {
        b.item[i] = search1_args(*cur[i], refs[i], *nets[i], level, src_idx, net_width);
        maxrefs = b.item[i].nrefs > maxrefs ? b.item[i].nrefs : maxrefs;
        totrefs += b.item[i].nrefs;
    }
    const int nblk = b.item[0].nblk;
    if (nblk <= 0 || maxrefs == 0 || search1_skip()) return;
    if (search1_split((size_t)nblk * totrefs, false))
        VP8_LAUNCH(k_search1_b<true>, dim3((nblk + S1Map<true>::BLOCKS_PER_WG - 1) / S1Map<true>::BLOCKS_PER_WG, maxrefs, n), dim3(256), 0, s, b);
    else if (search1_pre_lds() && search1_ref_loop())
        VP8_LAUNCH(k_search1_plr_b, dim3((nblk + S1Map<false>::BLOCKS_PER_WG - 1) / S1Map<false>::BLOCKS_PER_WG, 1, n), dim3(256), 0, s, b);
    else if (search1_pre_lds())
        VP8_LAUNCH(k_search1_pl_b, dim3((nblk + S1Map<false>::BLOCKS_PER_WG - 1) / S1Map<false>::BLOCKS_PER_WG, maxrefs, n), dim3(256), 0, s, b);
    else
        VP8_LAUNCH(k_search1_b<false>, dim3((nblk + S1Map<false>::BLOCKS_PER_WG - 1) / S1Map<false>::BLOCKS_PER_WG, maxrefs, n), dim3(256), 0, s, b);
}

__global__ __launch_bounds__(256) void k_weight_tap(const int32_t *d, int n, int32_t *out) {
    const int i = blockIdx.x * 256 + threadIdx.x;
    if (i >= n) return;
    uint32_t cc[4], pp[4];
#pragma unroll
    for (int c = 0; c < 4; ++c) {
        cc[c] = pp[c] = 0;
#pragma unroll
        for (int r = 0; r < 4; ++r) {
            const int v = d[i * 16 + 4 * r + c];
            const uint32_t cb = (uint32_t)(v > 0 ? v : 0) ^ 0x80u, pb = (uint32_t)(v > 0 ? 0 : -v) ^ 0x80u;
            cc[c] |= cb << (8 * r);
            pp[c] |= pb << (8 * r);
        }
    }
    int pre[16];
#pragma unroll
    for (int c = 0; c < 4; ++c) weight_pre_column(cc[c], pre + 4 * c);
    out[i] = weight_cols_pre(pre, pp);
}
void launch_weight_tap(hipStream_t s, const int32_t *d, int n, int32_t *out) {
    hipLaunchKernelGGL(k_weight_tap, dim3((n + 255) / 256), dim3(256), 0, s, d, n, out);
}
__global__ __attribute__((amdgpu_waves_per_eu(8, 8))) __launch_bounds__(256) void k_weight_tap_mfma(const int32_t *d, int n, int32_t *out) {
    const int i0 = blockIdx.x * 256 + threadIdx.x, i = i0 < n ? i0 : n - 1;
    uint32_t cc[4];
    v4i pp;
#pragma unroll
    for (int c = 0; c < 4; ++c) {
        uint32_t cw = 0, pw = 0;
#pragma unroll
        for (int r = 0; r < 4; ++r) {
            const int v = d[i * 16 + 4 * r + c];
            const uint32_t cb = (uint32_t)(v > 0 ? v : 0) ^ 0x80u, pb = (uint32_t)(v > 0 ? 0 : -v) ^ 0x80u;
            cw |= cb << (8 * r);
            pw |= pb << (8 * r);
        }
        cc[c] = cw;
        pp[c] = (int)pw;
    }
    int pre[16];
    weight_pre_block(cc, pre);
    v16i c16;
#pragma unroll
    for (int k = 0; k < 16; ++k) c16[k] = pre[k];
    const int w = weight_mfma(metric_a((int)threadIdx.x), c16, pp);
    if (i0 < n) out[i0] = w;
}
void launch_weight_tap_mfma(hipStream_t s, const int32_t *d, int n, int32_t *out) {
    hipLaunchKernelGGL(k_weight_tap_mfma, dim3((n + 255) / 256), dim3(256), 0, s, d, n, out);
}

}
```

### vp8oclenc_amd/csrc/lf_banded.h

```cpp
#pragma once
#include "lf_shared.h"

namespace vp8 {
namespace lfb {

using namespace lf;

constexpr int WORKERS = 4;
constexpr int ROWS = 2 * WORKERS;
constexpr int RING_MB = 16;
constexpr int SROW = RING_MB * 16;
constexpr int STRIP_PLANE = 4 * SROW;
constexpr int STRIP_BYTES = 3 * STRIP_PLANE;
constexpr int TILE_S = 24;
constexpr int TILE_PLANE = 16 * TILE_S;
constexpr int TILE_BYTES = 3 * TILE_PLANE;
constexpr int TILE_SLOTS = 2;
constexpr int NWAVES = WORKERS + 2;

enum { F_TOP = WORKERS, F_PUB, F_ABORT = 7 };

__device__ __forceinline__ uint32_t pack4(int a, int b, int c, int d) {
    const uint32_t lo = __builtin_amdgcn_perm((uint32_t)satb(b), (uint32_t)satb(a), 0x0c0c0400u);
    const uint32_t hi = __builtin_amdgcn_perm((uint32_t)satb(d), (uint32_t)satb(c), 0x0c0c0400u);
    return __builtin_amdgcn_perm(hi, lo, 0x05040100u);
}
__device__ __forceinline__ int ub(uint32_t w, int k) { return byte_of(w, k) | BIAS; }

__device__ __forceinline__ uint32_t ld_sc1(const uint32_t *p) {
    return __hip_atomic_load(p, __ATOMIC_RELAXED, __HIP_MEMORY_SCOPE_AGENT);
}
__device__ __forceinline__ void st_sc1(uint32_t *p, uint32_t v) {
    __hip_atomic_store(p, v, __ATOMIC_RELAXED, __HIP_MEMORY_SCOPE_AGENT);
}
constexpr int WAIT_LGKM0 = 0xc07f;
#define LF_WAIT(cond_unsatisfied, nap) LF_BOUNDED_WAIT(cond_unsatisfied, nap, false)

struct Args {
    Plane Y, U, V;
    MBOut o;
    SegData *sd;
    LfCheck chk;
    int32_t *gprog;
    int gbase;
    int mbw, mbh, nbands;
    int32_t *err;
};
static_assert(sizeof(BatchOf<Args>) <= 4096, "a batch's argument blocks travel in the 4 KiB kernel-argument segment");

template <typename Filter> struct Shared {
    uint8_t strip[ROWS + 1][STRIP_BYTES];
    uint8_t tile[ROWS][TILE_SLOTS][TILE_BYTES];
    int flag[8];
    uint32_t dummy[WORKERS * 64];
    SegData sd;
    float red[8];
    int repl;
    int first_lf0;
    typename Filter::Lim lim[4];
};

template <typename Filter> __device__ __forceinline__ void loop_filter_body(const Args &a) {
    __shared__ __attribute__((aligned(16))) Shared<Filter> sh;
    const int band = blockIdx.x;
    const int wave = __builtin_amdgcn_readfirstlane(threadIdx.x >> 6), lane = threadIdx.x & 63;
    lds_flag_t *const flag = (lds_flag_t *)sh.flag;
    if (threadIdx.x < 8) flag[threadIdx.x] = 0;
    if constexpr (Filter::LEVEL0_ENDS_PLANE) {
        if (threadIdx.x == 0) sh.first_lf0 = 0x7fffffff;
    }
    const int32_t *sdv = a.sd->v;
    if (a.chk.on) {
        sdv = check_ssim_segments<NWAVES>(a, sh, wave);
        if (band >= a.nbands) {
            static_assert(sizeof(sh.strip) + sizeof(sh.tile) >= VERDICT_CHUNK * sizeof(float), "staging area");
            verdict_workgroup<NWAVES>(a, sh, sdv != a.sd->v, reinterpret_cast<float *>(&sh.strip[0][0]));
            return;
        }
    } else if (band >= a.nbands) {
        return;
    }
    if (threadIdx.x < 4)
        sh.lim[threadIdx.x] = Filter::limits(sdv + threadIdx.x * SD_INTS);
    unsigned long long *clk = reinterpret_cast<unsigned long long *>(a.err + 4);
    if (band == 0 && threadIdx.x == 0) __hip_atomic_store(clk, __builtin_amdgcn_s_memrealtime(), __ATOMIC_RELAXED, __HIP_MEMORY_SCOPE_AGENT);
    const unsigned long long cyc0 = __builtin_amdgcn_s_memtime(), tick0 = __builtin_amdgcn_s_memrealtime();
    const uint32_t hwid0 = hw_slot();
    __syncthreads();
    const int mbw = a.mbw, mbh = a.mbh;
    const int band_row0 = band * ROWS;
    if constexpr (Filter::LEVEL0_ENDS_PLANE) {
        const bool any0 = sdv[SD_LOOP_FILTER_LEVEL] == 0 || sdv[SD_INTS + SD_LOOP_FILTER_LEVEL] == 0 ||
                          sdv[2 * SD_INTS + SD_LOOP_FILTER_LEVEL] == 0 || sdv[3 * SD_INTS + SD_LOOP_FILTER_LEVEL] == 0;
        if (any0) {
            int first = 0x7fffffff;
            for (int mb = threadIdx.x; mb < mbw * mbh; mb += NWAVES * 64)
                if (sdv[a.o.seg[mb] * SD_INTS + SD_LOOP_FILTER_LEVEL] == 0) { first = mb; break; }
            if (first != 0x7fffffff) atomicMin(&sh.first_lf0, first);
            __syncthreads();
        }
    }

    if (wave == WORKERS + 1) {
        if (band + 1 >= a.nbands) return;
        constexpr int STORE_LANES = Filter::CHROMA ? 44 : 20;
        const int pl = lane < 20 ? 0 : (lane < 32 ? 1 : 2);
        const int k = pl == 0 ? lane : (pl == 1 ? lane - 20 : lane - 32);
        const int ndw = pl == 0 ? 5 : 3;
        const int rr = k / ndw, j = k % ndw;
        const Plane &P = pl == 0 ? a.Y : (pl == 1 ? a.U : a.V);
        const int msz = pl == 0 ? 16 : 8, rmask = RING_MB * msz - 1;
        const int y = (band_row0 + ROWS - 1) * msz + (msz - 4) + rr;
        const uint8_t *sp = sh.strip[ROWS] + pl * STRIP_PLANE + rr * SROW;
        for (int x = 0; x <= mbw; ++x) {
            const int done = 2 * (x + ROWS - 1) + 2;
            LF_WAIT(flag[WORKERS - 1] < done, 3)
            if (lane < STORE_LANES) {
                const uint32_t v = *reinterpret_cast<const uint32_t *>(sp + ((x * msz - 4 + 4 * j) & rmask));
                st_sc1(reinterpret_cast<uint32_t *>(P.p + (ptrdiff_t)y * P.stride + x * msz - 4) + j, v);
            }
            asm volatile("s_waitcnt vmcnt(0)" ::: "memory");
            if (lane == 0) {
                flag[F_PUB] = x + 1;
                __hip_atomic_store(&a.gprog[band], a.gbase + x + 1, __ATOMIC_RELAXED, __HIP_MEMORY_SCOPE_AGENT);
            }
        }
        return;
    }

    if (wave == WORKERS) {
        if (band == 0) return;
        const int l = lane & 31;
        const int pl = l < 16 ? 0 : (l < 24 ? 1 : 2);
        const int k = pl == 0 ? l : (pl == 1 ? l - 16 : l - 24);
        const int nd = pl == 0 ? 4 : 2;
        const int r = k / nd, j = k % nd;
        const Plane &P = pl == 0 ? a.Y : (pl == 1 ? a.U : a.V);
        const int msz = pl == 0 ? 16 : 8, rmask = RING_MB * msz - 1;
        const int y = band_row0 * msz - 4 + r;
        uint8_t *sp = sh.strip[0] + pl * STRIP_PLANE + r * SROW;
        uint8_t *gp = P.p + (ptrdiff_t)y * P.stride + 4 * j;
        constexpr int DRAIN_LANES = Filter::CHROMA ? 32 : 16;
#define DRAIN_TOP(m)                                                                                        \
    {                                                                                                       \
        LF_WAIT(flag[0] < 2 * (m) + 2, 8)                                                                    \
        if (lane < DRAIN_LANES) st_sc1(reinterpret_cast<uint32_t *>(gp + (m) * msz - 4),                    \
                              *reinterpret_cast<const uint32_t *>(sp + (((m) * msz - 4 + 4 * j) & rmask))); \
    }
        for (int x = 0; x < mbw; ++x) {
            const int need = imin(x + 2, mbw + 1);
            LF_WAIT(__hip_atomic_load(&a.gprog[band - 1], __ATOMIC_RELAXED, __HIP_MEMORY_SCOPE_AGENT) - a.gbase < need, 2)
            if (x >= RING_MB - 1) DRAIN_TOP(x - (RING_MB - 1))
            if (lane < 32) *reinterpret_cast<uint32_t *>(sp + ((x * msz + 4 * j) & rmask)) = ld_sc1(reinterpret_cast<const uint32_t *>(gp + x * msz));
            lds_fence();
            if (lane == 0) flag[F_TOP] = x + 1;
        }
        for (int m = imax(mbw - (RING_MB - 1), 0); m <= mbw; ++m) DRAIN_TOP(m)
#undef DRAIN_TOP
        return;
    }

    __builtin_amdgcn_s_setprio(3);
    const int half = lane >> 5, l32 = lane & 31;
    const int r = 2 * wave + half;
    const int gr = band_row0 + r;
    const bool row_real = gr < mbh, row_any = gr <= mbh;
    const int pl = l32 < 16 ? 0 : (l32 < 24 ? 1 : 2);
    const int li = pl == 0 ? l32 : (pl == 1 ? l32 - 16 : l32 - 24);
    const int msz = pl == 0 ? 16 : 8, nd = msz / 4;
    const Plane &P = pl == 0 ? a.Y : (pl == 1 ? a.U : a.V);
    const int rmask = RING_MB * msz - 1;
    uint8_t *top = sh.strip[r] + pl * STRIP_PLANE;
    uint8_t *bot = sh.strip[r + 1] + pl * STRIP_PLANE;
    const bool bottom_lane = li >= msz - 4;
    uint8_t *botw = bottom_lane ? bot + (li - (msz - 4)) * SROW : reinterpret_cast<uint8_t *>(&sh.dummy[lane]);
    const int botw_mask = bottom_lane ? rmask : 0;
    const int tile_lane = pl * TILE_PLANE + li * TILE_S;
    const int tile_col = pl * TILE_PLANE + 4 + li;
    const bool from_top = li < 4;
    const bool drain_lane = (Filter::CHROMA || pl == 0) && row_any && (from_top ? gr > 0 && !(r == 0 && band > 0) : row_real);
    const uint8_t *dr_src = from_top ? top + li * SROW : sh.tile[r][0] + pl * TILE_PLANE + (li - 4) * TILE_S;
    const int dr_slot = from_top ? 0 : TILE_BYTES;
    const int dr_and = from_top ? rmask : 0xffff;
    const int dr_col = from_top ? -1 : 0;
    uint8_t *dr_g = P.p + (ptrdiff_t)(gr * msz - 4 + li) * P.stride - 4;
    const bool has_top = gr > 0;
    const bool publishes = band + 1 < a.nbands;
    [[maybe_unused]] int first_lf0 = 0x7fffffff;
    if constexpr (Filter::LEVEL0_ENDS_PLANE) first_lf0 = sh.first_lf0;
    const uint8_t *pf_p = P.p + (ptrdiff_t)(imin(gr, mbh - 1) * msz + li) * P.stride;
    const int32_t *pf_seg = a.o.seg + imin(gr, mbh - 1) * mbw, *pf_mask = a.o.mask + imin(gr, mbh - 1) * mbw;
    uint4 nxt = make_uint4(0, 0, 0, 0);
    int nxt_seg = 0, nxt_mask = 0;
    if (row_real) {
        nxt = *reinterpret_cast<const uint4 *>(pf_p);
        nxt_seg = pf_seg[0];
        nxt_mask = pf_mask[0];
    }
    uint32_t left4 = 0;
    const int steps = mbw + ROWS + 1;
    for (int S = 0; S < steps; ++S) {
        uint8_t *tile = sh.tile[r][S & 1];
        const int x = S - r;
        const bool p1_on = row_real & (x >= 0) & (x <= mbw);
        const bool mbstep = p1_on & (x < mbw);
        const int x0 = x * msz;
        int t[20];
#pragma unroll
        for (int k = 0; k < 16; ++k) t[4 + k] = ub(k < 4 ? nxt.x : (k < 8 ? nxt.y : (k < 12 ? nxt.z : nxt.w)), k & 3);
        const int seg = nxt_seg, maskv = nxt_mask;
        if (mbstep & (x + 1 < mbw)) {
            nxt = *reinterpret_cast<const uint4 *>(pf_p + x0 + msz);
            nxt_seg = pf_seg[x + 1];
            nxt_mask = pf_mask[x + 1];
        }
        if (drain_lane & (x >= 1) & (x <= mbw + 1)) {
            const int c0 = ((x - 1) * msz - 4) & dr_col;
            const uint8_t *src = dr_src + ((S - 1) & 1) * dr_slot;
            uint32_t v[4];
#pragma unroll
            for (int j = 0; j < 4; ++j) v[j] = *reinterpret_cast<const uint32_t *>(src + ((c0 + 4 * j) & dr_and));
            uint32_t *g = reinterpret_cast<uint32_t *>(dr_g + (x - 1) * msz);
            *reinterpret_cast<uint2 *>(g) = make_uint2(v[0], v[1]);
            if (pl == 0) *reinterpret_cast<uint2 *>(g + 2) = make_uint2(v[2], v[3]);
        }
        const typename Filter::Lim lim = sh.lim[seg & 3];
        bool do_filter = mbstep;
        if constexpr (Filter::LEVEL0_ENDS_PLANE) do_filter = mbstep & ((gr * mbw + x) < first_lf0);
        if constexpr (!Filter::CHROMA) do_filter = do_filter & (pl == 0);
        const typename Filter::Step fs = Filter::step(lim, do_filter & (maskv != 0), pl == 0);
        uint32_t *trow = reinterpret_cast<uint32_t *>(tile + tile_lane);
        if (p1_on) {
#pragma unroll
            for (int k = 0; k < 4; ++k) t[k] = ub(left4, k);
            Filter::line(t, fs, do_filter & (x > 0));
            const uint32_t d0 = pack4(t[0], t[1], t[2], t[3]);
            trow[0] = d0;
#pragma unroll
            for (int j = 1; j < 5; ++j) trow[j] = pack4(t[4 * j], t[4 * j + 1], t[4 * j + 2], t[4 * j + 3]);
            *reinterpret_cast<uint32_t *>(botw + ((x0 - 4) & botw_mask)) = d0;
        }
        __builtin_amdgcn_s_waitcnt(WAIT_LGKM0);
        flag[wave] = 2 * S + 1;
        {
            const int need_up = 2 * S + 1;
            const int need_dn = wave + 1 < WORKERS ? 2 * (S - (RING_MB - 3)) + 1 : 0;
            const int x_r0 = S - 2 * wave;
            const bool top_dep = wave == 0 && band > 0 && x_r0 >= 0 && x_r0 <= mbw && band_row0 <= mbh;
            const int need_top = imin(x_r0 + 1, mbw);
            const int need_pub = (wave + 1 == WORKERS && publishes) ? S - (ROWS - 1) - (RING_MB - 2) : 0;
            const int up = imax(wave - 1, 0), dn = imin(wave + 1, WORKERS - 1);
            for (int spins = 0;; ++spins) {
                const int f_up = flag[up], f_dn = flag[dn], f_top = flag[F_TOP], f_pub = flag[F_PUB], f_abort = flag[F_ABORT];
                const bool ok = (wave == 0 || f_up >= need_up) && (wave + 1 == WORKERS || f_dn >= need_dn) && (!top_dep || f_top >= need_top) &&
                                f_pub >= need_pub;
                const int state = __builtin_amdgcn_readfirstlane(f_abort ? 2 : (ok ? 1 : 0));
                if (state == 1) break;
                if (state == 2) return;
                if (spins > SPIN_LIMIT) { flag[F_ABORT] = 1; *a.err = 1; }
                if (spins < 32) asm volatile("s_nop 3"); else __builtin_amdgcn_s_sleep(1);
            }
        }
        if (mbstep) {
            int t[20];
            const int rc = (x0 + li) & rmask;
            uint8_t *tp = top + rc, *bp = bot + rc, *tc = tile + tile_col;
#pragma unroll
            for (int k = 0; k < 4; ++k) t[k] = (int)tp[k * SROW];
#pragma unroll
            for (int k = 0; k < 16; ++k) t[4 + k] = (int)tc[k * TILE_S];
            __builtin_amdgcn_s_waitcnt(WAIT_LGKM0);
#pragma unroll
            for (int k = 0; k < 20; ++k) t[k] |= BIAS;
            Filter::line(t, fs, do_filter & has_top);
            tp[1 * SROW] = (uint8_t)satb(t[1]); tp[2 * SROW] = (uint8_t)satb(t[2]); tp[3 * SROW] = (uint8_t)satb(t[3]);
            int s[16];
#pragma unroll
            for (int k = 0; k < 16; ++k) { s[k] = satb(t[4 + k]); tc[k * TILE_S] = (uint8_t)s[k]; }
#pragma unroll
            for (int j = 0; j < 4; ++j) bp[j * SROW] = (uint8_t)(pl == 0 ? s[12 + j] : s[4 + j]);
            left4 = trow[nd];
        }
        __builtin_amdgcn_s_waitcnt(WAIT_LGKM0);
        flag[wave] = 2 * S + 2;
    }
    if (gr == mbh && l32 == 0) {
        const unsigned long long t0 = __hip_atomic_load(clk, __ATOMIC_RELAXED, __HIP_MEMORY_SCOPE_AGENT);
        const unsigned long long t1 = __builtin_amdgcn_s_memrealtime();
        atomicAdd(clk + 1, t1 - t0);
        atomicAdd(clk + 2, 1ull);
        const unsigned long long ratio = (__builtin_amdgcn_s_memtime() - cyc0) * 1000ull / (t1 - tick0 + 1);
        LF_CLOCK_RATIO(clk, ratio, hwid0)
    }
}

inline Args make_args(hipStream_t s, const Frame &recon, const MBOut &o, SegData *d_sd, int32_t *progress, int counter_word, int mbw, int mbh,
                      unsigned launch_no, const LfCheck *chk) {
    Args a;
    if (chk) a.chk = *chk;
    else a.chk.on = 0;
    a.Y = recon.Y[0];
    a.U = recon.U;
    a.V = recon.V;
    a.o = o;
    a.sd = d_sd;
    a.gprog = progress + counter_word;
    a.mbw = mbw;
    a.mbh = mbh;
    a.nbands = (mbh + 1 + ROWS - 1) / ROWS;
    a.gbase = lf_window_base(launch_no, mbw);
    if (a.gbase == 0) (void)hipMemsetAsync(a.gprog, 0, sizeof(int32_t) * (a.nbands + 1), s);
    a.err = progress + LF_ERR_WORD;
    return a;
}

template <typename Kernel>
inline void launch_batch(Kernel kernel, hipStream_t s, const Frame *const *recon, const MBOut *const *o, SegData *const *d_sd, int32_t *const *progress,
                         int counter_word, int mbw, int mbh, const unsigned *launch_no, int n, const LfCheck *chk, bool skip = false) {
    BatchOf<Args> b;
    b.n = n;
    bool any = false;
    for (int i = 0; i < n; ++i) {
        b.item[i] = make_args(s, *recon[i], *o[i], d_sd[i], progress[i], counter_word, mbw, mbh, launch_no[i], chk ? &chk[i] : nullptr);
        any = any || b.item[i].chk.on;
    }
    if (skip) return;
    VP8_LAUNCH(kernel, dim3(b.item[0].nbands + (any ? 1 : 0), 1, n), dim3(NWAVES * 64), 0, s, b);
}

}
}
```

### vp8oclenc_amd/csrc/vp8hip_dev.h

```cpp
#pragma once
#include <hip/hip_runtime.h>
#include <hip/hip_ext.h>
#include <stdint.h>
#include <stdlib.h>
#include <string.h>

#include <vector>

#include "../../include/vp8hip.h"

namespace vp8 {

struct LaunchTiming { hipEvent_t start = nullptr, stop = nullptr; int launches = 0; };
extern thread_local LaunchTiming tl_timing;
#define VP8_LAUNCH(kernel, grid, block, shmem, stream, ...)                                                                               \
    do {                                                                                                                                  \
        ++::vp8::tl_timing.launches;                                                                                                      \
        hipExtLaunchKernelGGL(kernel, grid, block, shmem, stream, ::vp8::tl_timing.start, ::vp8::tl_timing.stop, 0, __VA_ARGS__);         \
    } while (0)

constexpr int PAD = 32;
constexpr int EXT = 8;
constexpr int LF_ERR_WORD = 1536;
constexpr int LF_SIMPLE_WORD = 512;
constexpr int LF_SIMPLE_WORDS = 512;
constexpr int S2_CLOCK_WORD = LF_ERR_WORD + 32;
constexpr int CLOCK_SAMPLE = 64;
constexpr int SD_INTS = 11;
enum { SD_Y_AC_I = 0, SD_Y_DC_IDELTA, SD_Y2_DC_IDELTA, SD_Y2_AC_IDELTA, SD_UV_DC_IDELTA, SD_UV_AC_IDELTA,
       SD_LOOP_FILTER_LEVEL, SD_MBEDGE_LIMIT, SD_SUB_BEDGE_LIMIT, SD_INTERIOR_LIMIT, SD_HEV_THRESHOLD };

struct Plane {
    uint8_t *p;
    int stride;
    int w, h;
};

struct Frame {
    Plane Y[5];
    Plane U, V;
};

struct RefSet {
    Frame ref[3];
    int use[3];
};

struct NetSet {
    int16_t *net[3][2];
    int32_t *bdiff[3];
};

struct MBOut {
    int32_t *parts, *ref, *seg, *nz, *mask;
    int16_t *vec;
    int16_t *coeffs;
    float *ssim;
    int32_t *flags;
};

struct SegData { int32_t v[4 * SD_INTS]; };

constexpr int MAX_BATCH = 8;
template <typename A> struct BatchOf { int n; A item[MAX_BATCH]; };

#if defined(__HIPCC__)
__device__ __forceinline__ bool launch_clock_sampled() {
    const unsigned wg = (blockIdx.z * gridDim.y + blockIdx.y) * gridDim.x + blockIdx.x;
    return wg % CLOCK_SAMPLE == 0;
}
__device__ __forceinline__ void launch_clock_begin(unsigned long long *w) {
    if (w && launch_clock_sampled() && __builtin_amdgcn_readfirstlane((int)threadIdx.x) == 0)
        atomicMin(&w[0], (unsigned long long)__builtin_amdgcn_s_memrealtime());
}
__device__ __forceinline__ void launch_clock_end(unsigned long long *w) {
    if (!w || !launch_clock_sampled()) return;
    __syncthreads();
    if (threadIdx.x != 0) return;
    atomicMax(&w[1], (unsigned long long)__builtin_amdgcn_s_memrealtime());
    __threadfence();
    const unsigned total = gridDim.x * gridDim.y * gridDim.z, sampled = (total + CLOCK_SAMPLE - 1) / CLOCK_SAMPLE;
    if (atomicAdd(&w[2], 1ull) + 1 == sampled) {
        __threadfence();
        const unsigned long long t1 = atomicExch(&w[1], 0ull), t0 = atomicExch(&w[0], ~0ull);
        atomicExch(&w[2], 0ull);
        atomicAdd(&w[3], t1 - t0);
        atomicAdd(&w[4], 1ull);
    }
}
#endif
#ifdef VP8HIP_EXPERIMENTS
inline bool experiment_skip(const char *what) { const char *v = getenv("VP8HIP_EXPERIMENT_SKIP"); return v && strstr(v, what) != nullptr; }
inline const char *experiment_env(const char *name) { return getenv(name); }
#else
inline bool experiment_skip(const char *) { return false; }
inline const char *experiment_env(const char *) { return nullptr; }
#endif
int persistent_workgroups();

void launch_border(hipStream_t s, const Frame &f);
void launch_pyramid(hipStream_t s, const Frame *a, const Frame *b, uint32_t border_mask = 0);
void launch_pack(hipStream_t s, const Frame &f, const void *y, const void *u, const void *v, int sw = 0, int sh = 0, int ssy = 0, int ssc = 0);
void launch_pyramid_batch(hipStream_t s, const Frame *const *f, int nframes, uint32_t border_mask = 0);
struct ScanRequest { uint32_t *partial, *stats; SegData *sd; int32_t *strength_out; int is_key; int32_t refqi[4]; int qi_min; };
void launch_pack_batch(hipStream_t s, const Frame *const *f, const void *const *y, const void *const *u, const void *const *v, int n,
                       int sw = 0, int sh = 0);
struct ScaleDim { int n, n_in, n_surf; size_t off_start, off_coef; int max_span[4]; };
struct ScalePlan { int in_w = 0, in_h = 0, kind = 0; ScaleDim d[4] = {}; uint8_t *d_blob = nullptr; };
bool scale_plan_make(ScalePlan *p, int in_w, int in_h, int dst_w, int dst_h, int W, int H, int kind, std::vector<uint8_t> &blob);
void launch_scale_batch(hipStream_t s, const Frame *const *f, const void *const *y, const void *const *u, const void *const *v,
                        const ScalePlan *const *plan, int n);
struct DenoiseMirror { int32_t frame_number, mbs_filtered, mbs_total; uint32_t seq; };
struct DenoiseItem { Frame cur, hist; unsigned long long *word; DenoiseMirror *host; uint32_t seq; int32_t frame_number; };
void launch_denoise_batch(hipStream_t s, const DenoiseItem *items, int n, int level);
bool launch_search1_coarse_batch(hipStream_t s, const Frame *const *cur, const RefSet *refs, const NetSet *const *nets, int net_width, int n, bool finest, bool top_only = false);
void launch_search1_batch(hipStream_t s, const Frame *const *cur, const RefSet *refs, const NetSet *const *nets, int level, int src_idx,
                          int net_width, int n);
bool launch_search2_batch(hipStream_t s, const Frame *const *cur, const RefSet *refs, const NetSet *const *nets, int n,
                          unsigned long long *clk = nullptr, const ScanRequest *const *scan = nullptr);
void launch_mb_batch(hipStream_t s, const Frame *const *cur, const RefSet *refs, const NetSet *const *nets, const Frame *const *recon,
                     const MBOut *const *o, const SegData *const *d_sd, float ssim_target, int mbw, int mbh, int n,
                     bool conformant = false);
struct LfCheck;
void launch_loop_filter3_batch(hipStream_t s, const Frame *const *recon, const MBOut *const *o, SegData *const *d_sd,
                               int32_t *const *progress, int mbw, int mbh, const unsigned *launch_no, int n, const LfCheck *chk = nullptr);
void launch_loop_filter4_batch(hipStream_t s, const Frame *const *recon, const MBOut *const *o, SegData *const *d_sd,
                               int32_t *const *progress, void *const *handoff, int mbw, int mbh, const unsigned *launch_no, int n,
                               const LfCheck *chk = nullptr);
void launch_auto_segments_batch(hipStream_t s, const Frame *const *cur, uint32_t *const *partial, uint32_t *const *stats, SegData *const *sd,
                                int32_t *const *strength_out, const int *is_key, const int32_t (*refqi)[4], int qi_min, int n);
void launch_search1_coarse(hipStream_t s, const Frame &cur, const RefSet &refs, const NetSet &nets, int net_width, bool finest);
void launch_search1(hipStream_t s, const Frame &cur, const RefSet &refs, const NetSet &nets, int level,
                    int src_idx, int net_width, bool latency = false);
void launch_search2(hipStream_t s, const Frame &cur, const RefSet &refs, const NetSet &nets, unsigned long long *clk = nullptr);
void launch_weight_tap(hipStream_t s, const int32_t *d, int n, int32_t *out);
void launch_weight_tap_mfma(hipStream_t s, const int32_t *d, int n, int32_t *out);
void launch_mb(hipStream_t s, const Frame &cur, const RefSet &refs, const NetSet &nets, const Frame &recon,
               const MBOut &o, const SegData *d_sd, float ssim_target, int mbw, int mbh, bool conformant = false);
void launch_filter_mask(hipStream_t s, const MBOut &o, const SegData *d_sd, int mbs);
void launch_loop_filter4(hipStream_t s, const Frame &recon, const MBOut &o, SegData *d_sd, int32_t *progress, void *handoff,
                         int mbw, int mbh, unsigned launch_no, int stall_test = 0, const LfCheck *chk = nullptr);
size_t loop_filter4_handoff_bytes(int mbw, int mbh);
void launch_loop_filter_simple(hipStream_t s, const Frame &recon, const MBOut &o, SegData *d_sd, int32_t *progress, int mbw, int mbh,
                               unsigned launch_no, const LfCheck *chk = nullptr);
void launch_loop_filter_simple_batch(hipStream_t s, const Frame *const *recon, const MBOut *const *o, SegData *const *d_sd,
                                     int32_t *const *progress, int mbw, int mbh, const unsigned *launch_no, int n, const LfCheck *chk = nullptr);
bool loop_filter_simple_fits(int mbh);

constexpr int QUALITY_TILE_COLS = 63;
constexpr int QUALITY_TILE_ROWS = 8;
struct QualitySums {
    int64_t frames;
    uint64_t sse[3], samples[3];
    double psnr_all_sum, ssim_all_sum, ssim_sum[3], psnr_min;
    int64_t psnr_min_frame;
};
struct QualityState {
    vp8hip_quality pending;
    int32_t has_pending;
    uint32_t seq;
    QualitySums sums;
};
struct QualityPartial { unsigned long long sse; double ssim; };
struct QualityPlane { const uint8_t *s, *r; int ss, rs, w, h; };
struct QualityArgs {
    QualityPlane p[3];
    QualityPartial *partial;
    unsigned *ticket;
    QualityState *state;
    QualityState *host;
    uint32_t seq;
    int32_t frame_number, is_key;
};
int quality_tiles(int w, int h);
QualityArgs quality_args(const Frame &src, const Frame &rec, int w, int h);
void launch_quality(hipStream_t s, const QualityArgs &a);
void launch_quality_batch(hipStream_t s, const QualityArgs *a, int n);
void quality_totals(const QualityState &st, vp8hip_quality_totals *t);

size_t rc_partial_words();
void launch_lf_strength(hipStream_t s, const Frame &cur, uint32_t *partial, uint32_t *stats);
void launch_chroma_sad(hipStream_t s, const Frame &cur, const Frame &prev, uint32_t *partial, uint32_t *stats);
void launch_auto_segments(hipStream_t s, const Frame &cur, uint32_t *partial, uint32_t *stats, SegData *sd, int32_t *strength_out,
                          int is_key, const int32_t refqi[4], int qi_min);

constexpr int ENT_NCTX = 4 * 8 * 3 * 11;
constexpr int ENT_MAX_PARTITIONS = 8;
#if !defined(VP8HIP_ENT_CHUNK)
#define VP8HIP_ENT_CHUNK 256
#endif
constexpr int ENT_CHUNK = VP8HIP_ENT_CHUNK;
void launch_ent_count(hipStream_t s, const MBOut &o, uint8_t *flags, uint8_t *third_ctx, uint32_t *counts, uint32_t *probs,
                      uint32_t *denom0, int mbw, int mbh, int num_partitions, const uint8_t *defaults = nullptr);
struct EntPlan {
    uint32_t bool_base[ENT_MAX_PARTITIONS + 1], chunk_base[ENT_MAX_PARTITIONS + 1], word_base[ENT_MAX_PARTITIONS + 1];
    uint32_t nbools[ENT_MAX_PARTITIONS], w_end[ENT_MAX_PARTITIONS], nbytes[ENT_MAX_PARTITIONS];
    uint32_t total_chunks, overflow;
};
struct EntBuffers {
    uint32_t *offs, *tile_sum;
    uint16_t *bools;
    uint32_t *maps;
    void *start;
    void *acc;
    uint8_t *bytes;
    int32_t *sizes;
    EntPlan *plan;
    uint32_t cap_bools, cap_chunks, cap_words;
};
void launch_ent_encode(hipStream_t s, const MBOut &o, const uint8_t *third_ctx, const uint32_t *probs, const EntBuffers &eb,
                       int mbw, int mbh, int P, bool code = true);

void launch_scan_exclusive(hipStream_t s, uint32_t *v, uint32_t *tile_sum, int n);
void launch_bool_code(hipStream_t s, const EntBuffers &eb, int P);
void launch_frame_code(hipStream_t s, const EntBuffers &coef, int P, const EntBuffers &hdr, uint32_t head, uint32_t capacity, uint8_t *frame);
inline size_t ent_maps_entries(uint32_t cap_chunks) { return ((size_t)cap_chunks + cap_chunks / 8 + 2 * ENT_MAX_PARTITIONS) * 128; }

struct HdrFrame { int is_key, is_golden, is_altref, loop_filter_type, sharpness , partitions_log2; };
void launch_default_probs(hipStream_t s, uint32_t *probs, const uint32_t *denom0);
const uint8_t *hdr_default_coeff_probs();
constexpr int HDR_STAT_WORDS = 84;
void launch_hdr_encode(hipStream_t s, const MBOut &o, const int32_t *is_inter, const int32_t *modes, const HdrFrame &f, const SegData *d_sd,
                       const int32_t *strength, const uint32_t *probs, const uint32_t *denom0, const EntBuffers &eb, uint32_t *partial,
                       uint8_t *sym, uint32_t *info, int mbw, int mbh, bool code = true);

struct FrameEntropy {
    MBOut o;
    uint8_t *flags, *third;
    uint32_t *counts, *probs, *denom0;
    const EntBuffers *coef, *hdr;
    uint32_t *hdr_partial, *hdr_info;
    uint8_t *hdr_sym;
    const int32_t *is_inter, *modes;
    HdrFrame f;
    const SegData *d_sd;
    const int32_t *strength;
    int mbw, mbh, P;
};
void launch_fe_count(hipStream_t s, const FrameEntropy &e);
void launch_fe_emit(hipStream_t s, const FrameEntropy &e);
struct FrameOut { uint8_t *frame; uint32_t head, capacity; };
void launch_fe_count_batch(hipStream_t s, const FrameEntropy *e, int n);
void launch_fe_emit_batch(hipStream_t s, const FrameEntropy *e, int n);
void launch_frame_code_batch(hipStream_t s, const FrameEntropy *e, const FrameOut *fo, int n);

void launch_intra(hipStream_t s, const Frame &cur, const Frame &recon, const MBOut &o, const SegData *d_sd, int32_t *modes,
                  int32_t *is_inter, int32_t *prog, unsigned gen, int32_t *err, float target, int key, int mbw, int mbh, int stall_test = 0,
                  int modes_of_kept = 0);
void launch_ssim_stats(hipStream_t s, const MBOut &o, const int32_t *is_inter, int mbs, const int32_t *err, int32_t *out);
struct CheckItem {
    const Frame *cur, *recon;
    const MBOut *o;
    const SegData *sd;
    int32_t *modes, *is_inter, *prog, *err;
    unsigned gen;
};
struct LfCheck {
    int on, qi_min;
    int32_t refqi[4];
    const int32_t *is_inter;
    int32_t *strength;
    int32_t *stats;
    int32_t *verdict;
    uint32_t seq;
};
void launch_check_fallback(hipStream_t s, const CheckItem *items, int n, float target, int mbw, int mbh, int modes_of_kept);
void launch_intra_key_batch(hipStream_t s, const CheckItem *items, int n, int mbw, int mbh);

#if defined(__HIPCC__)
__device__ __forceinline__ int iabs(int v) { return v < 0 ? -v : v; }
__device__ __forceinline__ int sat8(int v) { return v < 0 ? 0 : (v > 255 ? 255 : v); }
__device__ __forceinline__ int imin(int a, int b) { return a < b ? a : b; }
__device__ __forceinline__ int imax(int a, int b) { return a > b ? a : b; }
__device__ __forceinline__ int iclamp(int v, int lo, int hi) { return v < lo ? lo : (v > hi ? hi : v); }
__device__ __forceinline__ int byte_of(uint32_t w, int k) { return (int)((w >> (8 * k)) & 0xffu); }

__device__ __forceinline__ int xcd_band(int x, int n) {
#if defined(VP8HIP_NO_XCD_BANDS)
    (void)n;
    return x;
#else
    const int k = x & 7, chunk = n >> 3, rem = n & 7;
    return k * chunk + (k < rem ? k : rem) + (x >> 3);
#endif
}

static __device__ __constant__ const int k_dc_q[128] = {
    4,   5,   6,   7,   8,   9,   10,  10,  11,  12,  13,  14,  15,  16,  17,  17,  18,  19,  20,  20,  21,  21,
    22,  22,  23,  23,  24,  25,  25,  26,  27,  28,  29,  30,  31,  32,  33,  34,  35,  36,  37,  37,  38,  39,
    40,  41,  42,  43,  44,  45,  46,  46,  47,  48,  49,  50,  51,  52,  53,  54,  55,  56,  57,  58,  59,  60,
    61,  62,  63,  64,  65,  66,  67,  68,  69,  70,  71,  72,  73,  74,  75,  76,  76,  77,  78,  79,  80,  81,
    82,  83,  84,  85,  86,  87,  88,  89,  91,  93,  95,  96,  98,  100, 101, 102, 104, 106, 108, 110, 112, 114,
    116, 118, 122, 124, 126, 128, 130, 132, 134, 136, 138, 140, 143, 145, 148, 151, 154, 157};
static __device__ __constant__ const int k_ac_q[128] = {
    4,   5,   6,   7,   8,   9,   10,  11,  12,  13,  14,  15,  16,  17,  18,  19,  20,  21,  22,  23,  24,  25,
    26,  27,  28,  29,  30,  31,  32,  33,  34,  35,  36,  37,  38,  39,  40,  41,  42,  43,  44,  45,  46,  47,
    48,  49,  50,  51,  52,  53,  54,  55,  56,  57,  58,  60,  62,  64,  66,  68,  70,  72,  74,  76,  78,  80,
    82,  84,  86,  88,  90,  92,  94,  96,  98,  100, 102, 104, 106, 108, 110, 112, 114, 116, 119, 122, 125, 128,
    131, 134, 137, 140, 143, 146, 149, 152, 155, 158, 161, 164, 167, 170, 173, 177, 181, 185, 189, 193, 197, 201,
    205, 209, 213, 217, 221, 225, 229, 234, 239, 245, 249, 254, 259, 264, 269, 274, 279, 284};
__device__ __forceinline__ int qi(int v) { return iclamp(v, 0, 127); }

__device__ __forceinline__ int fill_segment_data(SegData *sd, int is_key, const int refqi[4], int qi_min, int reductor, int sharpness,
                                                 bool update_filter) {
    if (update_filter) { reductor *= 2; sharpness = 7; }
    int32_t *v = sd->v;
    for (int i = 0; i < 4 * SD_INTS; ++i) v[i] = 0;
    v[SD_Y_DC_IDELTA] = 15;
    v[SD_UV_DC_IDELTA] = is_key ? 0 : -15;
    v[SD_UV_AC_IDELTA] = is_key ? 0 : -15;
    for (int i = 0; i < 4; ++i) {
        int32_t *s = v + SD_INTS * i;
        s[SD_Y_AC_I] = is_key ? qi_min : refqi[i];
        const int y_dc_q = k_dc_q[qi(s[SD_Y_AC_I] + v[SD_Y_DC_IDELTA])];
        int lvl = y_dc_q / reductor;
        lvl = lvl > 63 ? 63 : (lvl < 0 ? 0 : lvl);
        s[SD_LOOP_FILTER_LEVEL] = lvl;
        int il = lvl;
        if (sharpness) {
            il >>= sharpness > 4 ? 2 : 1;
            if (il > 9 - sharpness) il = 9 - sharpness;
        }
        if (!il) il = 1;
        s[SD_INTERIOR_LIMIT] = il;
        s[SD_MBEDGE_LIMIT] = ((lvl + 2) * 2) + il;
        s[SD_SUB_BEDGE_LIMIT] = (lvl * 2) + il;
        int hev = 0;
        if (is_key) hev = lvl >= 40 ? 2 : (lvl >= 15 ? 1 : 0);
        else hev = lvl >= 40 ? 3 : (lvl >= 20 ? 2 : (lvl >= 15 ? 1 : 0));
        s[SD_HEV_THRESHOLD] = hev;
    }
    return sharpness;
}

__device__ __forceinline__ uint32_t ld_u32(const uint8_t *p) {
    uint32_t v;
    __builtin_memcpy(&v, p, 4);
    return v;
}
__device__ __forceinline__ uint2 ld_u64(const uint8_t *p) {
    uint2 v;
    __builtin_memcpy(&v, p, 8);
    return v;
}

typedef short s16x2 __attribute__((ext_vector_type(2)));
__device__ __forceinline__ uint32_t pk16(int lo, int hi) { return __builtin_amdgcn_perm((uint32_t)hi, (uint32_t)lo, 0x05040100u); }
__device__ __forceinline__ int dot2(uint32_t xy, uint32_t k, int c) {
    return __builtin_amdgcn_sdot2(__builtin_bit_cast(s16x2, xy), __builtin_bit_cast(s16x2, k), c, true);
}
constexpr uint32_t K_ROT_A = 2217u | (5352u << 16);
constexpr uint32_t K_ROT_B = (uint32_t)(-5352 & 0xffff) | (2217u << 16);

typedef unsigned short u16x2 __attribute__((ext_vector_type(2)));
__device__ __forceinline__ s16x2 as_s16x2(uint32_t v) { return __builtin_bit_cast(s16x2, v); }
__device__ __forceinline__ uint32_t as_u32(s16x2 v) { return __builtin_bit_cast(uint32_t, v); }
__device__ __forceinline__ uint32_t abs_acc(s16x2 v, uint32_t acc) {
    return __builtin_amdgcn_sad_u16(as_u32(v) ^ 0x80008000u, 0x80008000u, acc);
}

constexpr uint32_t pk8s(int a, int b, int c, int d) {
    return (uint32_t)(a & 255) | ((uint32_t)(b & 255) << 8) | ((uint32_t)(c & 255) << 16) | ((uint32_t)(d & 255) << 24);
}
constexpr uint32_t K_W_R0 = pk8s(8, 8, -8, 8), K_W_R2 = pk8s(8, -8, 8, 8), K_W_X = pk8s(0, 0, 16, 0), K_W_Y = pk8s(32, 0, 0, -32);
constexpr uint32_t K_W_R0N = pk8s(-8, -8, 8, -8), K_W_R2N = pk8s(-8, 8, -8, -8), K_W_XN = pk8s(0, 0, -16, 0), K_W_YN = pk8s(-32, 0, 0, 32);
constexpr uint32_t K_ROT16_A = 2217u | (21408u << 16);
constexpr uint32_t K_ROT16_B = (uint32_t)(-5352 & 0xffff) | (8868u << 16);
__device__ __forceinline__ int dot4s(uint32_t a, uint32_t k, int c) { return __builtin_amdgcn_sdot4((int)a, (int)k, c, true); }

__device__ __forceinline__ void weight_pre_column(uint32_t ccol, int pre[4]) {
    pre[0] = dot4s(ccol, K_W_R0, 0);
    pre[1] = dot4s(ccol, K_W_R2, 0);
    pre[2] = dot4s(ccol, K_W_X, 0);
    pre[3] = dot4s(ccol, K_W_Y, 0);
}

__device__ __forceinline__ uint32_t weight_rows_tail(uint32_t o0, uint32_t o2, uint32_t xy_lo, uint32_t xy_hi, uint32_t d1, uint32_t acc) {
    const int t1l = dot2(xy_lo, K_ROT_A, 12000 + (1 << 28)), t1h = dot2(xy_hi, K_ROT_A, 12000 + (1 << 28));
    const int t3l = dot2(xy_lo, K_ROT_B, 51000 + (1 << 28)), t3h = dot2(xy_hi, K_ROT_B, 51000 + (1 << 28));
    const uint32_t o1 = __builtin_amdgcn_perm((uint32_t)t1h, (uint32_t)t1l, 0x07060302u);
    const uint32_t o3 = __builtin_amdgcn_perm((uint32_t)t3h, (uint32_t)t3l, 0x07060302u);
    uint32_t ones = 0x00010001u;
    asm("" : "+s"(ones));
    const uint32_t nz = __builtin_bit_cast(uint32_t, __builtin_elementwise_min(__builtin_bit_cast(u16x2, d1), __builtin_bit_cast(u16x2, ones)));
    acc = __builtin_amdgcn_sad_u16(o0, 0x08000800u, acc);
    acc = __builtin_amdgcn_sad_u16(o1, 0x10001000u - nz, acc);
    acc = __builtin_amdgcn_sad_u16(o2, 0x08000800u, acc);
    return __builtin_amdgcn_sad_u16(o3, 0x10001000u, acc);
}
__device__ __forceinline__ int weight_rows_end(uint32_t acc, uint32_t o00) {
    const int a00 = (int)__builtin_amdgcn_sad_u16(o00 & 0xffffu, 2048u, 0u);
    return (int)acc - (a00 - (a00 >> 2));
}
__device__ __forceinline__ int weight_rows(const s16x2 A[4], const s16x2 B[4]) {
    uint32_t acc = 0, o00 = 0;
#pragma unroll
    for (int h = 0; h < 2; ++h) {
        const s16x2 *X = h == 0 ? A : B;
        const s16x2 a1 = X[0] + X[3], d1 = X[0] - X[3], b1 = X[1] + X[2], c1 = X[1] - X[2];
        const u16x2 a7 = __builtin_bit_cast(u16x2, a1) + u16x2{0x8007, 0x8007};
        const u16x2 o0 = (a7 + __builtin_bit_cast(u16x2, b1)) >> u16x2{4, 4};
        const u16x2 o2 = (a7 - __builtin_bit_cast(u16x2, b1)) >> u16x2{4, 4};
        const uint32_t xy_lo = __builtin_amdgcn_perm(as_u32(d1), as_u32(c1), 0x05040100u);
        const uint32_t xy_hi = __builtin_amdgcn_perm(as_u32(d1), as_u32(c1), 0x07060302u);
        acc = weight_rows_tail(__builtin_bit_cast(uint32_t, o0), __builtin_bit_cast(uint32_t, o2), xy_lo, xy_hi, as_u32(d1), acc);
        if (h == 0) o00 = __builtin_bit_cast(uint32_t, o0);
    }
    return weight_rows_end(acc, o00);
}

__device__ __forceinline__ int weight_cols_pre(const int pre[16], const uint32_t p[4]) {
    s16x2 A[4], B[4];
#pragma unroll
    for (int c = 0; c < 4; ++c) {
        const int R0 = dot4s(p[c], K_W_R0N, pre[4 * c + 0]);
        const int R2 = dot4s(p[c], K_W_R2N, pre[4 * c + 1]);
        const int X = dot4s(p[c], K_W_XN, pre[4 * c + 2]);
        const int Y = dot4s(p[c], K_W_YN, pre[4 * c + 3]);
        const uint32_t xy = pk16(X, Y);
        const int t1 = dot2(xy, K_ROT16_A, 16 * 14500);
        const int t3 = dot2(xy, K_ROT16_B, 16 * 7500);
        A[c] = as_s16x2(__builtin_amdgcn_perm((uint32_t)t1, (uint32_t)R0, 0x07060100u));
        B[c] = as_s16x2(__builtin_amdgcn_perm((uint32_t)t3, (uint32_t)R2, 0x07060100u));
    }
    return weight_rows(A, B);
}

typedef int v4i __attribute__((ext_vector_type(4)));
typedef int v16i __attribute__((ext_vector_type(16)));
enum { METRIC_S0, METRIC_M0, METRIC_C0, METRIC_D0, METRIC_S2, METRIC_M2, METRIC_C2, METRIC_D2, METRIC_X , METRIC_Y = 12  };
constexpr uint32_t metric_w(int i, int c) {
    if (i >= METRIC_X) return (i & 3) != c ? 0u : i >= METRIC_Y ? K_W_YN : K_W_XN;
    const uint32_t pos = i < METRIC_S2 ? K_W_R0N : K_W_R2N, neg = i < METRIC_S2 ? K_W_R0 : K_W_R2;
    switch (i & 3) {
    case METRIC_S0: return pos;
    case METRIC_M0: return c == 0 || c == 3 ? pos : neg;
    case METRIC_C0: return c == 1 ? pos : c == 2 ? neg : 0u;
    default: return c == 0 ? pos : c == 3 ? neg : 0u;
    }
}
struct MetricTable { uint32_t w[64][4]; };
constexpr MetricTable make_metric_a() {
    MetricTable t{};
    for (int l = 0; l < 64; ++l) {
        const int m = l & 31, h = l >> 5;
        if (((m >> 2) & 1) != h) continue;
        const int i = (m & 3) + 4 * (m >> 3);
        for (int c = 0; c < 4; ++c) t.w[l][c] = metric_w(i, c);
    }
    return t;
}
static __device__ __constant__ const MetricTable K_METRIC_A = make_metric_a();
__device__ __forceinline__ v4i metric_a(int wave_lane) { return *reinterpret_cast<const v4i *>(K_METRIC_A.w[wave_lane & 63]); }

__device__ __forceinline__ void weight_pre_half(const uint32_t cc[4], uint32_t k_r, uint32_t k_xy, int smcd[4], int xy[4]) {
    int R[4];
#pragma unroll
    for (int c = 0; c < 4; ++c) {
        R[c] = dot4s(cc[c], k_r, 0);
        xy[c] = dot4s(cc[c], k_xy, 0);
    }
    const int a7 = R[0] + R[3] + 0x8007, b = R[1] + R[2];
    smcd[METRIC_S0] = a7 + b;
    smcd[METRIC_M0] = a7 - b;
    smcd[METRIC_C0] = R[1] - R[2];
    smcd[METRIC_D0] = R[0] - R[3];
}
__device__ __forceinline__ void weight_pre_block(const uint32_t cc[4], int pre[16]) {
    weight_pre_half(cc, K_W_R0, K_W_X, pre + METRIC_S0, pre + METRIC_X);
    weight_pre_half(cc, K_W_R2, K_W_Y, pre + METRIC_S2, pre + METRIC_Y);
}

__device__ __forceinline__ int weight_mfma(v4i a, v16i c, v4i p) {
    const v16i d = __builtin_amdgcn_mfma_i32_32x32x32_i8(a, p, c, 0, 0, 0);
    s16x2 P[4];
#pragma unroll
    for (int col = 0; col < 4; ++col) {
        const uint32_t xy = pk16(d[METRIC_X + col], d[METRIC_Y + col]);
        const int t1 = dot2(xy, K_ROT16_A, 16 * 14500);
        const int t3 = dot2(xy, K_ROT16_B, 16 * 7500);
        P[col] = as_s16x2(__builtin_amdgcn_perm((uint32_t)t3, (uint32_t)t1, 0x07060302u));
    }
    uint32_t acc = 0;
    {
        const s16x2 a1 = P[0] + P[3], d1 = P[0] - P[3], b1 = P[1] + P[2], c1 = P[1] - P[2];
        const u16x2 a7 = __builtin_bit_cast(u16x2, a1) + u16x2{0x8007, 0x8007};
        const u16x2 o0 = (a7 + __builtin_bit_cast(u16x2, b1)) >> u16x2{4, 4};
        const u16x2 o2 = (a7 - __builtin_bit_cast(u16x2, b1)) >> u16x2{4, 4};
        const uint32_t xy_lo = __builtin_amdgcn_perm(as_u32(d1), as_u32(c1), 0x05040100u);
        const uint32_t xy_hi = __builtin_amdgcn_perm(as_u32(d1), as_u32(c1), 0x07060302u);
        acc = weight_rows_tail(__builtin_bit_cast(uint32_t, o0), __builtin_bit_cast(uint32_t, o2), xy_lo, xy_hi, as_u32(d1), acc);
    }
    const u16x2 o0 = __builtin_bit_cast(u16x2, pk16(d[METRIC_S0], d[METRIC_S2])) >> u16x2{4, 4};
    const u16x2 o2 = __builtin_bit_cast(u16x2, pk16(d[METRIC_M0], d[METRIC_M2])) >> u16x2{4, 4};
    acc = weight_rows_tail(__builtin_bit_cast(uint32_t, o0), __builtin_bit_cast(uint32_t, o2), pk16(d[METRIC_C0], d[METRIC_D0]),
                           pk16(d[METRIC_C2], d[METRIC_D2]), pk16(d[METRIC_D0], d[METRIC_D2]), acc);
    return weight_rows_end(acc, __builtin_bit_cast(uint32_t, o0));
}
__device__ __forceinline__ v16i load_pre16(const int *pre16) {
    v16i c;
#pragma unroll
    for (int j = 0; j < 4; ++j) {
        const v4i v = *reinterpret_cast<const v4i *>(pre16 + 4 * j);
        c[4 * j] = v.x; c[4 * j + 1] = v.y; c[4 * j + 2] = v.z; c[4 * j + 3] = v.w;
    }
    return c;
}


__device__ __forceinline__ void transpose4x4(const uint32_t r[4], uint32_t c[4]) {
    const uint32_t t0 = __builtin_amdgcn_perm(r[1], r[0], 0x05010400u);
    const uint32_t t1 = __builtin_amdgcn_perm(r[1], r[0], 0x07030602u);
    const uint32_t t2 = __builtin_amdgcn_perm(r[3], r[2], 0x05010400u);
    const uint32_t t3 = __builtin_amdgcn_perm(r[3], r[2], 0x07030602u);
    c[0] = __builtin_amdgcn_perm(t2, t0, 0x05040100u);
    c[1] = __builtin_amdgcn_perm(t2, t0, 0x07060302u);
    c[2] = __builtin_amdgcn_perm(t3, t1, 0x05040100u);
    c[3] = __builtin_amdgcn_perm(t3, t1, 0x07060302u);
}

static __device__ __constant__ const int8_t k_sixtap[8][8] = {
    {0, 0, 127, 0, 0, 0, 0, 0},
    {0, -6, 123, 12, -1, 0, 0, 0},   {2, -11, 108, 36, -8, 1, 0, 0}, {0, -9, 93, 50, -6, 0, 0, 0},
    {3, -16, 77, 77, -16, 3, 0, 0},  {0, -6, 50, 93, -9, 0, 0, 0},   {1, -8, 36, 108, -11, 2, 0, 0},
    {0, -1, 12, 123, -6, 0, 0, 0},
};
__device__ __forceinline__ void load_taps(int phase, int f[6]) {
#pragma unroll
    for (int t = 0; t < 6; ++t) f[t] = k_sixtap[phase][t];
    if (phase == 0) f[2] = 128;
}
__device__ __forceinline__ int sat8_shr7(int s) { return iclamp(s, 0, 32767) >> 7; }
__device__ __forceinline__ int div128(int s) { return (s + ((s >> 31) & 127)) >> 7; }
#endif

}
```

Measured before the change: 71.72 million.

## Build reference and source pyramids inside loop-filter and pack kernels as rider blocks

Moves the downsampling pyramid and border extension into extra rider blocks. For the reconstructed reference they ride on the banded loop-filter kernel and wait on per-band done flags. For the current frame they ride on the pack kernel. This marks the pyramid and border as valid so the separate pyramid/border launches before motion estimation can be skipped. The cost is extra blocks that spin-wait on global progress words, more kernel arguments, and a release/fence signalling step in each loop-filter wave.

```diff
diff --git a/vp8oclenc_amd/build.py b/vp8oclenc_amd/build.py
--- a/vp8oclenc_amd/build.py
+++ b/vp8oclenc_amd/build.py
@@ -8,7 +8,7 @@
 CSRC = os.path.join(PKG, "csrc")
 LIB = os.path.join(PKG, "libvp8hip.so")
 SOURCES = ["api_context.hip", "api_inter.hip", "api_entropy.hip", "api_batch.hip", "api_shard.hip", "api_profile.hip", "kernels_me.hip", "kernels_scale.hip", "kernels_denoise.hip", "api_denoise.hip", "kernels_s2.hip", "kernels_mb.hip", "kernels_lf3.hip", "kernels_lf4.hip", "kernels_lf_simple.hip", "kernels_quality.hip", "api_quality.hip", "kernels_entropy_stage.hip", "kernels_rc.hip", "kernels_intra.hip", "vp8_host.cpp", "vp8_driver.cpp", "vp8_bitstream.cpp"]
-HEADERS = ["vp8hip_ctx.h", "vp8hip_dev.h", "kernels_rc_dev.h", "lf_shared.h", "lf_banded.h", "vp8_rfc6386_tables.inc", "vp8_mbhdr.h", "kernels_ent.hip", "kernels_hdr.hip"]
+HEADERS = ["vp8hip_ctx.h", "vp8hip_dev.h", "kernels_rc_dev.h", "lf_shared.h", "lf_banded.h", "pyramid_tile.h", "vp8_rfc6386_tables.inc", "vp8_mbhdr.h", "kernels_ent.hip", "kernels_hdr.hip"]
 HEADERS = HEADERS + [os.path.join("..", "..", "include", h) for h in ("vp8hip.h", "vp8hip_multi.h", "vp8hip_taps.h", "vp8hip_host.h", "vp8hip_driver.h", "vp8hip_bitstream.h")]
 
 
diff --git a/vp8oclenc_amd/csrc/api_batch.hip b/vp8oclenc_amd/csrc/api_batch.hip
--- a/vp8oclenc_amd/csrc/api_batch.hip
+++ b/vp8oclenc_amd/csrc/api_batch.hip
@@ -234,7 +234,10 @@
     {
         Timed t(c0, VP8HIP_K_PACK);
         if (c0->scale.in_w) launch_scale_batch(ps, f, py, pu, pv, plans, n);
-        else launch_pack_batch(ps, f, py, pu, pv, n, c0->src_w, c0->src_h);
+        else if (launch_pack_batch(ps, f, py, pu, pv, n, c0->src_w, c0->src_h, !c0->dn_level)) {
+            for (int i = 0; i < b->n; ++i)
+                if (!active || active[i]) b->c[i]->cur_pyramid_valid = true;
+        }
     }
     {
         DenoiseItem dn[MAX_BATCH];
@@ -449,6 +452,7 @@
     void *hand[MAX_BATCH];
     unsigned launch_no[MAX_BATCH];
     LfCheck chk[MAX_BATCH];
+    int ride[MAX_BATCH];
     int n = 0, type = -1;
     for (int i = 0; i < b->n; ++i) {
         if (active && !active[i]) continue;
@@ -466,23 +470,24 @@
         hand[n] = c->d_lf_handoff;
         launch_no[n] = type == 1 ? c->lf_simple_launches++ : c->lf_launches++;
         lf_check(c, chk[n]);
+        ride[n] = c->recon_key ? 0 : 1;
         c->verdict_stream = b->stream;
         m[n++] = c;
     }
     if (!n) return VP8HIP_OK;
+    bool rode = false;
     if (b->ent) HIPCHK(c0, hipEventRecord(b->ev_ent_fork, b->stream));
     {
         Timed t(c0, VP8HIP_K_LOOP_FILTER);
         static const bool form4 = [] { const char *v = getenv("VP8HIP_LF_BATCH_FORM"); return v && atoi(v) == 4; }();
         if (type == 1) launch_loop_filter_simple_batch(b->stream, recon, outs, sds, prog, c0->mbw, c0->mbh, launch_no, n, chk);
         else if (form4) launch_loop_filter4_batch(b->stream, recon, outs, sds, prog, hand, c0->mbw, c0->mbh, launch_no, n, chk);
-        else launch_loop_filter3_batch(b->stream, recon, outs, sds, prog, c0->mbw, c0->mbh, launch_no, n, chk);
+        else rode = launch_loop_filter3_batch(b->stream, recon, outs, sds, prog, c0->mbw, c0->mbh, launch_no, n, chk, ride);
     }
     b->ent_fork_fresh = b->ent != nullptr;
     for (int i = 0; i < n; ++i) {
         vp8hip_ctx *c = m[i];
-        c->frames[c->recon].pyramid_valid = false;
-        c->frames[c->recon].border_valid = false;
+        c->frames[c->recon].pyramid_valid = c->frames[c->recon].border_valid = rode && ride[i];
         c->slot[0] = c->recon;
         c->lf_key = c->recon_key;
         c->recon = -1;
diff --git a/vp8oclenc_amd/csrc/api_profile.hip b/vp8oclenc_amd/csrc/api_profile.hip
--- a/vp8oclenc_amd/csrc/api_profile.hip
+++ b/vp8oclenc_amd/csrc/api_profile.hip
@@ -131,6 +131,47 @@
             break;
         default:
             return VP8HIP_ERR_ARG;
+    }
+    HIPCHK(c, hipStreamSynchronize(s));
+    return VP8HIP_OK;
+}
+
+int vp8hip_debug_last_reference(vp8hip_ctx *c, int fresh, void *dst, size_t bytes, int32_t *valid) {
+    USE_DEVICE(c);
+    JOIN_LF(c);
+    if (!c || !dst) return VP8HIP_ERR_ARG;
+    if (c->slot[0] < 0) return VP8HIP_ERR_STATE;
+    hipStream_t s = c->stream;
+    const FrameSurf &last = c->frames[c->slot[0]];
+    if (valid) *valid = last.pyramid_valid && last.border_valid;
+    const Frame *f = &last.f;
+    if (fresh) {
+        const int idx = pick_free_frame(c);
+        if (idx < 0) return VP8HIP_ERR_STATE;
+        Frame &g = c->frames[idx].f;
+        const Plane *from[3] = {&f->Y[0], &f->U, &f->V}, *to[3] = {&g.Y[0], &g.U, &g.V};
+        for (int k = 0; k < 3; ++k)
+            HIPCHK(c, hipMemcpy2DAsync(to[k]->p, to[k]->stride, from[k]->p, from[k]->stride, from[k]->w, from[k]->h, hipMemcpyDeviceToDevice, s));
+        launch_pyramid(s, &g, nullptr, 1u);
+        c->frames[idx].pyramid_valid = false;
+        f = &g;
+    }
+    const Plane *padded[3] = {&f->Y[0], &f->U, &f->V};
+    size_t need = 0;
+    for (int k = 0; k < 3; ++k) need += (size_t)(padded[k]->w + 2 * EXT) * (padded[k]->h + 2 * EXT);
+    for (int l = 1; l <= 4; ++l) need += (size_t)f->Y[l].w * f->Y[l].h;
+    if (bytes != need) return VP8HIP_ERR_ARG;
+    uint8_t *d = static_cast<uint8_t *>(dst);
+    for (int k = 0; k < 3; ++k) {
+        const Plane &p = *padded[k];
+        const int w = p.w + 2 * EXT, h = p.h + 2 * EXT;
+        HIPCHK(c, hipMemcpy2DAsync(d, w, p.p - (ptrdiff_t)EXT * p.stride - EXT, p.stride, w, h, hipMemcpyDeviceToHost, s));
+        d += (size_t)w * h;
+    }
+    for (int l = 1; l <= 4; ++l) {
+        const int rc = copy_out(c, d, f->Y[l]);
+        if (rc) return rc;
+        d += (size_t)f->Y[l].w * f->Y[l].h;
     }
     HIPCHK(c, hipStreamSynchronize(s));
     return VP8HIP_OK;
diff --git a/vp8oclenc_amd/csrc/kernels_lf3.hip b/vp8oclenc_amd/csrc/kernels_lf3.hip
--- a/vp8oclenc_amd/csrc/kernels_lf3.hip
+++ b/vp8oclenc_amd/csrc/kernels_lf3.hip
@@ -9,6 +9,7 @@
 struct NormalFilter {
     static constexpr bool CHROMA = true;
     static constexpr bool LEVEL0_ENDS_PLANE = true;
+    static constexpr bool PYRAMID_RIDER = true;
     typedef int4 Lim;
     static __device__ __forceinline__ Lim limits(const int32_t *sd) {
         const int il = sd[SD_INTERIOR_LIMIT] & 0xff;
@@ -37,9 +38,10 @@
     return skip;
 }
 
-void launch_loop_filter3_batch(hipStream_t s, const Frame *const *recon, const MBOut *const *o, SegData *const *d_sd,
-                               int32_t *const *progress, int mbw, int mbh, const unsigned *launch_no, int n, const LfCheck *chk) {
-    lfb::launch_batch(lf3::k_loop_filter3_b, s, recon, o, d_sd, progress, 0, mbw, mbh, launch_no, n, chk, lf_skip());
+bool launch_loop_filter3_batch(hipStream_t s, const Frame *const *recon, const MBOut *const *o, SegData *const *d_sd,
+                               int32_t *const *progress, int mbw, int mbh, const unsigned *launch_no, int n, const LfCheck *chk, const int *ride) {
+    lfb::launch_batch(lf3::k_loop_filter3_b, s, recon, o, d_sd, progress, 0, mbw, mbh, launch_no, n, chk, lf_skip(), ride);
+    return !lf_skip();
 }
 
 }
diff --git a/vp8oclenc_amd/csrc/kernels_lf_simple.hip b/vp8oclenc_amd/csrc/kernels_lf_simple.hip
--- a/vp8oclenc_amd/csrc/kernels_lf_simple.hip
+++ b/vp8oclenc_amd/csrc/kernels_lf_simple.hip
@@ -23,6 +23,7 @@
 struct SimpleFilter {
     static constexpr bool CHROMA = false;
     static constexpr bool LEVEL0_ENDS_PLANE = false;
+    static constexpr bool PYRAMID_RIDER = false;
     typedef int2 Lim;
     static __device__ __forceinline__ Lim limits(const int32_t *sd) {
         const bool on = sd[SD_LOOP_FILTER_LEVEL] != 0;
diff --git a/vp8oclenc_amd/csrc/kernels_me.hip b/vp8oclenc_amd/csrc/kernels_me.hip
--- a/vp8oclenc_amd/csrc/kernels_me.hip
+++ b/vp8oclenc_amd/csrc/kernels_me.hip
@@ -2,22 +2,11 @@
 #include <string.h>
 
 #include "vp8hip_dev.h"
+#include "pyramid_tile.h"
 
 namespace vp8 {
 
 struct BorderItem { Plane y, u, v; };
-static_assert(EXT == 8, "border_row stores a margin as one eight-byte word");
-__device__ __forceinline__ void border_row(const Plane &pl, int row, int lane) {
-    if (row >= pl.h + EXT) return;
-    uint8_t *dst = pl.p + (ptrdiff_t)row * pl.stride;
-    const uint8_t *src = pl.p + (ptrdiff_t)iclamp(row, 0, pl.h - 1) * pl.stride;
-    if (row < 0 || row >= pl.h)
-        for (int x = lane * 8; x < pl.w; x += 512) *reinterpret_cast<uint2 *>(dst + x) = *reinterpret_cast<const uint2 *>(src + x);
-    if (lane < 2) {
-        const uint32_t s4 = (uint32_t)src[lane ? pl.w - 1 : 0] * 0x01010101u;
-        *reinterpret_cast<uint2 *>(dst + (lane ? pl.w : -EXT)) = make_uint2(s4, s4);
-    }
-}
 __device__ __forceinline__ void border_body(const BorderItem &a) {
     border_row(blockIdx.y == 0 ? a.y : (blockIdx.y == 1 ? a.u : a.v), (int)blockIdx.x - EXT, threadIdx.x);
 }
@@ -33,10 +22,9 @@
 static int border_jobs(const Frame &f) { return (f.Y[0].h + 2 * EXT) + 2 * (f.U.h + 2 * EXT); }
 
 __global__ __launch_bounds__(256) void k_pyramid(PyrArgs a) {
-    __shared__ uint8_t s2[16][16];
-    __shared__ uint8_t s3[8][8];
+    __shared__ PyrTileLds sh;
     const Frame &f = a.f[blockIdx.z];
-    const int t = threadIdx.x, tx = t & 15, ty = t >> 4;
+    const int t = threadIdx.x;
     const Plane &P0 = f.Y[0];
     const int tiles_y = (P0.h + 63) / 64;
     const int tile = xcd_band((int)blockIdx.y * (int)gridDim.x + (int)blockIdx.x, tiles_y * (int)gridDim.x);
@@ -50,48 +38,7 @@
         else if (job < ny + 2 * nc) border_row(f.V, job - ny - nc - EXT, t & 63);
         return;
     }
-    const int sx = imin(bx * 64 + 4 * tx, P0.w - 4), sy0 = by * 64 + 4 * ty;
-    uint32_t r[4];
-#pragma unroll
-    for (int k = 0; k < 4; ++k)
-        r[k] = *reinterpret_cast<const uint32_t *>(P0.p + (ptrdiff_t)imin(sy0 + k, P0.h - 1) * P0.stride + sx);
-    int l1[2][2];
-#pragma unroll
-    for (int j = 0; j < 2; ++j)
-#pragma unroll
-        for (int i = 0; i < 2; ++i)
-            l1[j][i] = (byte_of(r[2 * j], 2 * i) + byte_of(r[2 * j], 2 * i + 1) + byte_of(r[2 * j + 1], 2 * i) +
-                        byte_of(r[2 * j + 1], 2 * i + 1) + 2) >> 2;
-    const Plane &P1 = f.Y[1];
-    const int x1 = bx * 32 + 2 * tx, y1 = by * 32 + 2 * ty;
-    if (x1 < P1.w) {
-#pragma unroll
-        for (int j = 0; j < 2; ++j)
-            if (y1 + j < P1.h)
-                *reinterpret_cast<uint16_t *>(P1.p + (ptrdiff_t)(y1 + j) * P1.stride + x1) = (uint16_t)(l1[j][0] | (l1[j][1] << 8));
-    }
-    const int l2 = (l1[0][0] + l1[0][1] + l1[1][0] + l1[1][1] + 2) >> 2;
-    const Plane &P2 = f.Y[2];
-    const int x2 = bx * 16 + tx, y2 = by * 16 + ty;
-    if (x2 < P2.w && y2 < P2.h) P2.p[(ptrdiff_t)y2 * P2.stride + x2] = (uint8_t)l2;
-    s2[ty][tx] = (uint8_t)l2;
-    __syncthreads();
-    if (t < 64) {
-        const int ux = t & 7, uy = t >> 3;
-        const int l3 = (s2[2 * uy][2 * ux] + s2[2 * uy][2 * ux + 1] + s2[2 * uy + 1][2 * ux] + s2[2 * uy + 1][2 * ux + 1] + 2) >> 2;
-        const Plane &P3 = f.Y[3];
-        const int x3 = bx * 8 + ux, y3 = by * 8 + uy;
-        if (x3 < P3.w && y3 < P3.h) P3.p[(ptrdiff_t)y3 * P3.stride + x3] = (uint8_t)l3;
-        s3[uy][ux] = (uint8_t)l3;
-    }
-    __syncthreads();
-    if (t < 16) {
-        const int ux = t & 3, uy = t >> 2;
-        const int l4 = (s3[2 * uy][2 * ux] + s3[2 * uy][2 * ux + 1] + s3[2 * uy + 1][2 * ux] + s3[2 * uy + 1][2 * ux + 1] + 2) >> 2;
-        const Plane &P4 = f.Y[4];
-        const int x4 = bx * 4 + ux, y4 = by * 4 + uy;
-        if (x4 < P4.w && y4 < P4.h) P4.p[(ptrdiff_t)y4 * P4.stride + x4] = (uint8_t)l4;
-    }
+    pyramid_tile(P0, f.Y + 1, bx, by, t, true, sh);
 }
 
 static dim3 pyramid_grid(const Frame &f, int nframes, uint32_t border_mask) {
@@ -114,7 +61,8 @@
     VP8_LAUNCH(k_pyramid, pyramid_grid(*f[0], nframes, border_mask), dim3(256), 0, s, p);
 }
 
-struct PackItem { Plane py, pu, pv; const uint8_t *sy, *su, *sv; int sw, sh, ssy, ssc; };
+struct PackItem { Plane py, pu, pv; const uint8_t *sy, *su, *sv; int sw, sh, ssy, ssc; Plane lv[4]; int ride; };
+constexpr int PACK_TILES = 4;
 __device__ __forceinline__ void pack_body(const PackItem &a, int per) {
     const Plane &py = a.py, &pu = a.pu, &pv = a.pv;
     const uint8_t *sy = a.sy, *su = a.su, *sv = a.sv;
@@ -148,7 +96,22 @@
     }
 }
 
-__global__ __launch_bounds__(256) void k_pack_b(BatchOf<PackItem> b, int per) { pack_body(b.item[blockIdx.z], per); }
+__device__ __forceinline__ void pack_pyramid_tiles(const PackItem &a, int first) {
+    __shared__ PyrTileLds sh;
+    if (!a.ride) return;
+    const Plane src{const_cast<uint8_t *>(a.sy), a.ssy, a.sw, a.sh};
+    const int gx = (a.py.w + 63) / 64, ntiles = gx * ((a.py.h + 63) / 64);
+    for (int k = 0; k < PACK_TILES; ++k) {
+        const int tile = first * PACK_TILES + k;
+        if (tile >= ntiles) return;
+        pyramid_tile(src, a.lv, tile % gx, tile / gx, threadIdx.x, true, sh);
+    }
+}
+
+__global__ __launch_bounds__(256) void k_pack_b(BatchOf<PackItem> b, int per, int pack_blocks) {
+    if ((int)blockIdx.x >= pack_blocks) pack_pyramid_tiles(b.item[blockIdx.z], (int)blockIdx.x - pack_blocks);
+    else pack_body(b.item[blockIdx.z], per);
+}
 static int pack_units_per_thread() {
     static const int per = [] { const char *e = getenv("VP8HIP_PACK_UNITS"); const int v = e ? atoi(e) : 16; return v < 1 ? 1 : (v > 64 ? 64 : v); }();
     return per;
@@ -157,7 +120,10 @@
 static PackItem pack_item(const Frame &f, const void *y, const void *u, const void *v, int sw, int sh, int ssy, int ssc) {
     if (sw <= 0) { sw = f.Y[0].w; sh = f.Y[0].h; }
     if (ssy <= 0) { ssy = sw; ssc = sw >> 1; }
-    return PackItem{f.Y[0], f.U, f.V, (const uint8_t *)y, (const uint8_t *)u, (const uint8_t *)v, sw, sh, ssy, ssc};
+    return PackItem{f.Y[0], f.U, f.V, (const uint8_t *)y, (const uint8_t *)u, (const uint8_t *)v, sw, sh, ssy, ssc, {f.Y[1], f.Y[2], f.Y[3], f.Y[4]}, 0};
+}
+static bool pack_source_serves_pyramid(const PackItem &a) {
+    return a.sw == a.py.w && a.sh >= 1 && a.sh <= a.py.h && (a.ssy & 3) == 0 && (reinterpret_cast<uintptr_t>(a.sy) & 3) == 0;
 }
 void launch_pack(hipStream_t s, const Frame &f, const void *y, const void *u, const void *v, int sw, int sh, int ssy, int ssc) {
     const int n = (f.Y[0].w >> 3) * f.Y[0].h + 2 * ((f.U.w >> 3) * f.U.h);
@@ -165,18 +131,27 @@
     b.n = 1;
     b.item[0] = pack_item(f, y, u, v, sw, sh, ssy, ssc);
     const int per = pack_units_per_thread();
-    VP8_LAUNCH(k_pack_b, dim3((n + 256 * per - 1) / (256 * per), 1, 1), dim3(256), 0, s, b, per);
-}
-void launch_pack_batch(hipStream_t s, const Frame *const *f, const void *const *y, const void *const *u, const void *const *v, int n,
-                       int sw, int sh) {
+    const int blocks = (n + 256 * per - 1) / (256 * per);
+    VP8_LAUNCH(k_pack_b, dim3(blocks, 1, 1), dim3(256), 0, s, b, per, blocks);
+}
+bool launch_pack_batch(hipStream_t s, const Frame *const *f, const void *const *y, const void *const *u, const void *const *v, int n,
+                       int sw, int sh, bool with_pyramid) {
     BatchOf<PackItem> b;
     b.n = n;
-    for (int i = 0; i < n; ++i) b.item[i] = pack_item(*f[i], y[i], u[i], v[i], sw, sh, 0, 0);
+    for (int i = 0; i < n; ++i) {
+        b.item[i] = pack_item(*f[i], y[i], u[i], v[i], sw, sh, 0, 0);
+        with_pyramid = with_pyramid && pack_source_serves_pyramid(b.item[i]);
+    }
+    for (int i = 0; i < n; ++i) b.item[i].ride = with_pyramid ? 1 : 0;
     const int units = (f[0]->Y[0].w >> 3) * f[0]->Y[0].h + 2 * ((f[0]->U.w >> 3) * f[0]->U.h);
     static const bool skip = experiment_skip("pack");
-    if (skip) return;
+    if (skip) return false;
     const int per = pack_units_per_thread();
-    VP8_LAUNCH(k_pack_b, dim3((units + 256 * per - 1) / (256 * per), 1, n), dim3(256), 0, s, b, per);
+    const int blocks = (units + 256 * per - 1) / (256 * per);
+    const int tiles = ((f[0]->Y[0].w + 63) / 64) * ((f[0]->Y[0].h + 63) / 64);
+    const int riders = with_pyramid ? (tiles + PACK_TILES - 1) / PACK_TILES : 0;
+    VP8_LAUNCH(k_pack_b, dim3(blocks + riders, 1, n), dim3(256), 0, s, b, per, blocks);
+    return with_pyramid;
 }
 
 struct Search1Args {
diff --git a/vp8oclenc_amd/csrc/lf_banded.h b/vp8oclenc_amd/csrc/lf_banded.h
--- a/vp8oclenc_amd/csrc/lf_banded.h
+++ b/vp8oclenc_amd/csrc/lf_banded.h
@@ -1,5 +1,6 @@
 #pragma once
 #include "lf_shared.h"
+#include "pyramid_tile.h"
 
 namespace vp8 {
 namespace lfb {
@@ -45,6 +46,10 @@
     int gbase;
     int mbw, mbh, nbands;
     int32_t *err;
+    Plane pyr[4];
+    int32_t *gdone;
+    int tag;
+    int ride, rider0;
 };
 static_assert(sizeof(BatchOf<Args>) <= 4096, "a batch's argument blocks travel in the 4 KiB kernel-argument segment");
 
@@ -60,12 +65,64 @@
     typename Filter::Lim lim[4];
 };
 
+static_assert((ROWS * 16) % 128 == 0 && WORKERS + 1 <= LF_DONE_INTS, "a band is a whole number of pairs of tile rows; a word per signalling wave");
+constexpr int RIDER_NAP = 32;
+
+__device__ __forceinline__ void signal_done(const Args &a, int band, int slot, int lane) {
+    asm volatile("s_waitcnt vmcnt(0)" ::: "memory");
+    __builtin_amdgcn_fence(__ATOMIC_RELEASE, "agent");
+    asm volatile("s_waitcnt vmcnt(0)" ::: "memory");
+    if (lane == 0) __hip_atomic_store(&a.gdone[band * LF_DONE_INTS + slot], a.tag, __ATOMIC_RELAXED, __HIP_MEMORY_SCOPE_AGENT);
+}
+
+template <typename Filter> __device__ __forceinline__ void pyramid_rider(const Args &a, Shared<Filter> &sh, int k) {
+    static_assert(sizeof(sh.strip) >= sizeof(PyrTileLds), "the tile's LDS lies in the strips");
+    lds_flag_t *const flag = (lds_flag_t *)sh.flag;
+    const int wave = __builtin_amdgcn_readfirstlane(threadIdx.x >> 6), lane = threadIdx.x & 63;
+    const int tile_rows = (a.Y.h + 63) / 64;
+    if (!a.ride || k >= tile_rows) return;
+    const int band = k >> 1;
+    __syncthreads();
+    if (wave == 0) {
+        const bool lower_half = (k & 1) && band + 1 < a.nbands;
+        const bool polls = lane < WORKERS || (lane == WORKERS && lower_half);
+        const int32_t *w = a.gdone + (lane < WORKERS ? band * LF_DONE_INTS + lane : (band + 1) * LF_DONE_INTS + WORKERS);
+        for (int spins = 0;; ++spins) {
+            const int v = polls ? __hip_atomic_load(w, __ATOMIC_RELAXED, __HIP_MEMORY_SCOPE_AGENT) : a.tag;
+            if (!__any(v != a.tag)) break;
+            if (spins > SPIN_LIMIT / 8) { flag[F_ABORT] = 1; *a.err = 1; break; }
+            __builtin_amdgcn_s_sleep(RIDER_NAP);
+        }
+        __builtin_amdgcn_fence(__ATOMIC_ACQUIRE, "agent");
+        asm volatile("s_waitcnt vmcnt(0)" ::: "memory");
+    }
+    __syncthreads();
+    if (flag[F_ABORT]) return;
+    PyrTileLds &lds = *reinterpret_cast<PyrTileLds *>(&sh.strip[0][0]);
+    const int t = threadIdx.x, tiles_x = (a.Y.w + 63) / 64;
+    for (int bx = 0; bx < tiles_x; ++bx) pyramid_tile(a.Y, a.pyr, bx, k, t, t < 256, lds);
+    const bool first = k == 0, last = k + 1 == tile_rows;
+    const int y0 = first ? -EXT : k * 64, y1 = last ? a.Y.h + EXT : k * 64 + 64;
+    for (int y = y0 + wave; y < y1; y += NWAVES) border_row(a.Y, y, lane);
+    const int c0 = first ? -EXT : k * 32, c1 = last ? a.U.h + EXT : k * 32 + 32;
+    for (int y = c0 + wave; y < c1; y += NWAVES) {
+        border_row(a.U, y, lane);
+        border_row(a.V, y, lane);
+    }
+}
+
 template <typename Filter> __device__ __forceinline__ void loop_filter_body(const Args &a) {
     __shared__ __attribute__((aligned(16))) Shared<Filter> sh;
     const int band = blockIdx.x;
     const int wave = __builtin_amdgcn_readfirstlane(threadIdx.x >> 6), lane = threadIdx.x & 63;
     lds_flag_t *const flag = (lds_flag_t *)sh.flag;
     if (threadIdx.x < 8) flag[threadIdx.x] = 0;
+    if constexpr (Filter::PYRAMID_RIDER) {
+        if (band >= a.rider0) {
+            pyramid_rider<Filter>(a, sh, band - a.rider0);
+            return;
+        }
+    }
     if constexpr (Filter::LEVEL0_ENDS_PLANE) {
         if (threadIdx.x == 0) sh.first_lf0 = 0x7fffffff;
     }
@@ -157,6 +214,9 @@
         }
         for (int m = imax(mbw - (RING_MB - 1), 0); m <= mbw; ++m) DRAIN_TOP(m)
 #undef DRAIN_TOP
+        if constexpr (Filter::PYRAMID_RIDER) {
+            if (a.ride) signal_done(a, band, WORKERS, lane);
+        }
         return;
     }
 
@@ -284,6 +344,9 @@
         __builtin_amdgcn_s_waitcnt(WAIT_LGKM0);
         flag[wave] = 2 * S + 2;
     }
+    if constexpr (Filter::PYRAMID_RIDER) {
+        if (a.ride) signal_done(a, band, wave, lane);
+    }
     if (gr == mbh && l32 == 0) {
         const unsigned long long t0 = __hip_atomic_load(clk, __ATOMIC_RELAXED, __HIP_MEMORY_SCOPE_AGENT);
         const unsigned long long t1 = __builtin_amdgcn_s_memrealtime();
@@ -311,22 +374,33 @@
     a.gbase = lf_window_base(launch_no, mbw);
     if (a.gbase == 0) (void)hipMemsetAsync(a.gprog, 0, sizeof(int32_t) * (a.nbands + 1), s);
     a.err = progress + LF_ERR_WORD;
+    for (int l = 0; l < 4; ++l) a.pyr[l] = recon.Y[l + 1];
+    a.gdone = progress + LF_DONE_WORD;
+    a.tag = (int)(launch_no % 0x7ffffffeu) + 1;
+    a.ride = 0;
+    a.rider0 = 0x7fffffff;
     return a;
 }
 
 template <typename Kernel>
 inline void launch_batch(Kernel kernel, hipStream_t s, const Frame *const *recon, const MBOut *const *o, SegData *const *d_sd, int32_t *const *progress,
-                         int counter_word, int mbw, int mbh, const unsigned *launch_no, int n, const LfCheck *chk, bool skip = false) {
+                         int counter_word, int mbw, int mbh, const unsigned *launch_no, int n, const LfCheck *chk, bool skip = false,
+                         const int *ride = nullptr) {
     BatchOf<Args> b;
     b.n = n;
-    bool any = false;
+    bool any = false, riders = false;
     for (int i = 0; i < n; ++i) {
         b.item[i] = make_args(s, *recon[i], *o[i], d_sd[i], progress[i], counter_word, mbw, mbh, launch_no[i], chk ? &chk[i] : nullptr);
         any = any || b.item[i].chk.on;
+        b.item[i].ride = ride && ride[i] ? 1 : 0;
+        riders = riders || b.item[i].ride;
     }
     if (skip) return;
-    VP8_LAUNCH(kernel, dim3(b.item[0].nbands + (any ? 1 : 0), 1, n), dim3(NWAVES * 64), 0, s, b);
-}
-
-}
-}
+    const int rider0 = b.item[0].nbands + (any ? 1 : 0);
+    for (int i = 0; i < n; ++i) b.item[i].rider0 = rider0;
+    const int tile_rows = riders ? (recon[0]->Y[0].h + 63) / 64 : 0;
+    VP8_LAUNCH(kernel, dim3(rider0 + tile_rows, 1, n), dim3(NWAVES * 64), 0, s, b);
+}
+
+}
+}
diff --git a/vp8oclenc_amd/csrc/pyramid_tile.h b/vp8oclenc_amd/csrc/pyramid_tile.h
--- /dev/null
+++ b/vp8oclenc_amd/csrc/pyramid_tile.h
@@ -0,0 +1,69 @@
+#pragma once
+#include "vp8hip_dev.h"
+
+namespace vp8 {
+
+static_assert(EXT == 8, "border_row stores a margin as one eight-byte word");
+__device__ __forceinline__ void border_row(const Plane &pl, int row, int lane) {
+    if (row >= pl.h + EXT) return;
+    uint8_t *dst = pl.p + (ptrdiff_t)row * pl.stride;
+    const uint8_t *src = pl.p + (ptrdiff_t)iclamp(row, 0, pl.h - 1) * pl.stride;
+    if (row < 0 || row >= pl.h)
+        for (int x = lane * 8; x < pl.w; x += 512) *reinterpret_cast<uint2 *>(dst + x) = *reinterpret_cast<const uint2 *>(src + x);
+    if (lane < 2) {
+        const uint32_t s4 = (uint32_t)src[lane ? pl.w - 1 : 0] * 0x01010101u;
+        *reinterpret_cast<uint2 *>(dst + (lane ? pl.w : -EXT)) = make_uint2(s4, s4);
+    }
+}
+
+struct PyrTileLds { uint8_t s2[16][16]; uint8_t s3[8][8]; };
+
+__device__ __forceinline__ void pyramid_tile(const Plane &P0, const Plane *lv, int bx, int by, int t, bool on, PyrTileLds &sh) {
+    const int tx = t & 15, ty = (t >> 4) & 15;
+    if (on) {
+        const int sx = imin(bx * 64 + 4 * tx, P0.w - 4), sy0 = by * 64 + 4 * ty;
+        uint32_t r[4];
+#pragma unroll
+        for (int k = 0; k < 4; ++k)
+            r[k] = *reinterpret_cast<const uint32_t *>(P0.p + (ptrdiff_t)imin(sy0 + k, P0.h - 1) * P0.stride + sx);
+        int l1[2][2];
+#pragma unroll
+        for (int j = 0; j < 2; ++j)
+#pragma unroll
+            for (int i = 0; i < 2; ++i)
+                l1[j][i] = (byte_of(r[2 * j], 2 * i) + byte_of(r[2 * j], 2 * i + 1) + byte_of(r[2 * j + 1], 2 * i) +
+                            byte_of(r[2 * j + 1], 2 * i + 1) + 2) >> 2;
+        const Plane &P1 = lv[0];
+        const int x1 = bx * 32 + 2 * tx, y1 = by * 32 + 2 * ty;
+        if (x1 < P1.w) {
+#pragma unroll
+            for (int j = 0; j < 2; ++j)
+                if (y1 + j < P1.h)
+                    *reinterpret_cast<uint16_t *>(P1.p + (ptrdiff_t)(y1 + j) * P1.stride + x1) = (uint16_t)(l1[j][0] | (l1[j][1] << 8));
+        }
+        const int l2 = (l1[0][0] + l1[0][1] + l1[1][0] + l1[1][1] + 2) >> 2;
+        const Plane &P2 = lv[1];
+        const int x2 = bx * 16 + tx, y2 = by * 16 + ty;
+        if (x2 < P2.w && y2 < P2.h) P2.p[(ptrdiff_t)y2 * P2.stride + x2] = (uint8_t)l2;
+        sh.s2[ty][tx] = (uint8_t)l2;
+    }
+    __syncthreads();
+    if (t < 64) {
+        const int ux = t & 7, uy = t >> 3;
+        const int l3 = (sh.s2[2 * uy][2 * ux] + sh.s2[2 * uy][2 * ux + 1] + sh.s2[2 * uy + 1][2 * ux] + sh.s2[2 * uy + 1][2 * ux + 1] + 2) >> 2;
+        const Plane &P3 = lv[2];
+        const int x3 = bx * 8 + ux, y3 = by * 8 + uy;
+        if (x3 < P3.w && y3 < P3.h) P3.p[(ptrdiff_t)y3 * P3.stride + x3] = (uint8_t)l3;
+        sh.s3[uy][ux] = (uint8_t)l3;
+    }
+    __syncthreads();
+    if (t < 16) {
+        const int ux = t & 3, uy = t >> 2;
+        const int l4 = (sh.s3[2 * uy][2 * ux] + sh.s3[2 * uy][2 * ux + 1] + sh.s3[2 * uy + 1][2 * ux] + sh.s3[2 * uy + 1][2 * ux + 1] + 2) >> 2;
+        const Plane &P4 = lv[3];
+        const int x4 = bx * 4 + ux, y4 = by * 4 + uy;
+        if (x4 < P4.w && y4 < P4.h) P4.p[(ptrdiff_t)y4 * P4.stride + x4] = (uint8_t)l4;
+    }
+}
+
+}
diff --git a/vp8oclenc_amd/csrc/vp8hip_dev.h b/vp8oclenc_amd/csrc/vp8hip_dev.h
--- a/vp8oclenc_amd/csrc/vp8hip_dev.h
+++ b/vp8oclenc_amd/csrc/vp8hip_dev.h
@@ -24,6 +24,8 @@
 constexpr int LF_ERR_WORD = 1536;
 constexpr int LF_SIMPLE_WORD = 512;
 constexpr int LF_SIMPLE_WORDS = 512;
+constexpr int LF_DONE_WORD = 1792;
+constexpr int LF_DONE_INTS = 8;
 constexpr int S2_CLOCK_WORD = LF_ERR_WORD + 32;
 constexpr int CLOCK_SAMPLE = 64;
 constexpr int SD_INTS = 11;
@@ -103,8 +105,8 @@
 void launch_pack(hipStream_t s, const Frame &f, const void *y, const void *u, const void *v, int sw = 0, int sh = 0, int ssy = 0, int ssc = 0);
 void launch_pyramid_batch(hipStream_t s, const Frame *const *f, int nframes, uint32_t border_mask = 0);
 struct ScanRequest { uint32_t *partial, *stats; SegData *sd; int32_t *strength_out; int is_key; int32_t refqi[4]; int qi_min; };
-void launch_pack_batch(hipStream_t s, const Frame *const *f, const void *const *y, const void *const *u, const void *const *v, int n,
-                       int sw = 0, int sh = 0);
+bool launch_pack_batch(hipStream_t s, const Frame *const *f, const void *const *y, const void *const *u, const void *const *v, int n,
+                       int sw = 0, int sh = 0, bool with_pyramid = false);
 struct ScaleDim { int n, n_in, n_surf; size_t off_start, off_coef; int max_span[4]; };
 struct ScalePlan { int in_w = 0, in_h = 0, kind = 0; ScaleDim d[4] = {}; uint8_t *d_blob = nullptr; };
 bool scale_plan_make(ScalePlan *p, int in_w, int in_h, int dst_w, int dst_h, int W, int H, int kind, std::vector<uint8_t> &blob);
@@ -122,8 +124,9 @@
                      const MBOut *const *o, const SegData *const *d_sd, float ssim_target, int mbw, int mbh, int n,
                      bool conformant = false);
 struct LfCheck;
-void launch_loop_filter3_batch(hipStream_t s, const Frame *const *recon, const MBOut *const *o, SegData *const *d_sd,
-                               int32_t *const *progress, int mbw, int mbh, const unsigned *launch_no, int n, const LfCheck *chk = nullptr);
+bool launch_loop_filter3_batch(hipStream_t s, const Frame *const *recon, const MBOut *const *o, SegData *const *d_sd,
+                               int32_t *const *progress, int mbw, int mbh, const unsigned *launch_no, int n, const LfCheck *chk = nullptr,
+                               const int *ride = nullptr);
 void launch_loop_filter4_batch(hipStream_t s, const Frame *const *recon, const MBOut *const *o, SegData *const *d_sd,
                                int32_t *const *progress, void *const *handoff, int mbw, int mbh, const unsigned *launch_no, int n,
                                const LfCheck *chk = nullptr);
```

After: 69.38 million. 3.3% lower.
